# ScissorJack-ever/AlayaLite

Hardware: AMD Instinct MI355X
Metric: QPS @ recall@10>=0.95, GIST-960 L2, 1M base / 1k queries (higher is better)
Workload: dtype f32

## Files before the change

### alayalite_amd/csrc/capi.cpp

```cpp
#include "../../include/alaya_hip.h"

#include <hip/hip_runtime_api.h>

#include <algorithm>
#include <cfloat>
#include <cmath>
#include <cstring>
#include <memory>
#include <mutex>
#include <stdexcept>
#include <limits>
#include <string>
#include <thread>
#include <vector>

#include "build_kernels.h"
#include "extend_kernels.h"
#include "graph_update.h"
#include "hnsw_build.h"
#include "flat_bound.h"
#include "flat_filtered_kernels.h"
#include "flat_kernels.h"
#include <cstdlib>
#include "screen_bound.h"
// ... 33 lines not shown
    g_last_error = e.what();
    return ALAYA_ERR_DEVICE;
  } catch (const std::exception &e) {
    g_last_error = e.what();
    return ALAYA_ERR_RUNTIME;
  }
}

struct DevBuf {
  void *ptr = nullptr;
  size_t bytes = 0;
  void reserve(size_t n) {
    if (n <= bytes) return;
    release();
    hip_check(hipMalloc(&ptr, std::max<size_t>(n, 256)), "hipMalloc");
    bytes = std::max<size_t>(n, 256);
  }
  void release() {
    if (ptr) (void)hipFree(ptr);
    ptr = nullptr;
    bytes = 0;
  }
  template <typename T>
  T *as() const {
    return static_cast<T *>(ptr);
  }
  ~DevBuf() { release(); }
};

uint32_t round_up32(uint32_t d) { return (d + 31u) / 32u * 32u; }

uint32_t ceil_log2(uint64_t v) {
  uint32_t l = 0;
  while ((1ull << l) < v) ++l;
  return l;
}

}

struct alaya_index {
  int device = 0;
  std::mutex mu;
  uint64_t n = 0;
  uint32_t dim = 0, stride = 0;
  int metric = ALAYA_METRIC_L2;
  bool generic = false;
  DevBuf base, valid;
  bool has_valid = false;
  bool has_graph = false;
  uint32_t R = 0, upper_R = 0, ep = 0, n_eps = 0;
  bool has_overlay = false, dedup = false;
  DevBuf l0, levels, upper_off, upper_edges, eps;
  uint64_t graph_n = 0;
  bool has_sq8 = false;
  int sq8_order = 2;
  uint32_t code_stride = 0;
  DevBuf codes, sq_min, sq_max, rr_q_buf, sq_ids, sq_d;
  DevBuf norms, cand_d, cand_i, flat_tau, flag_buf, iota, flat_q;
  DevBuf flat_bias;
  int flat_contraction = -1;
  bool norms_ready = false;
  DevBuf flat_tiles, tiles_cand, tiles_qexp;
  bool tiles_ready = false;
  int tiles_exp = 0;
  int tiles_metric = -1;
  float max_norm = 0.f;
  DevBuf work, overflow, dirty, stab, q_buf, id_buf, dist_buf, cnt_buf, dlist_buf, dout_buf;
  DevBuf allow_buf, group_buf;
  DevBuf through_buf;
  DevBuf ff_ids, ff_sums, ff_count, ff_part_d, ff_part_i, ff_qlist;
  uint64_t ff_last[4] = {0, 0, 0, 0};
  size_t overflow_clean = 0;
  size_t stab_clean = 0;
  uint32_t hash_log2_override = 0;
  int helpers_mode = -1;
  DevBuf help_stats;
  uint64_t help_stats_slots = 0;
  struct ScreenCopy {
    DevBuf rows, err;
    uint64_t cap = 0;
    bool ready = false;
    bool failed = false;
  };
  ScreenCopy screen_copy[2];
  uint32_t screen_format = 0;
  DevBuf screen_stats;
  uint64_t screen_stats_slots = 0;
  uint32_t last_grid = 0, last_waves = 0;
  uint32_t last_lds = 0, last_hash_log2 = 0, last_compact = 0, last_per_cu = 0, last_scout = 0;
  DevBuf scout_stats;
  uint64_t scout_stats_slots = 0;
  DevBuf scout_policy_stats;
  uint32_t last_scout_policy = 0;
  int visited_mode_override = 0;
  int num_cus = 0;
  uint64_t capacity = 0;
  std::unique_ptr<alaya_amd::HostGraph> upd_graph;
  std::unique_ptr<alaya_amd::RowMirror> upd_rows;
  std::unique_ptr<alaya_amd::UpdateContext> upd_ctx;
  hipStream_t stream = nullptr;
  hipEvent_t scratch_ev = nullptr;
  hipStream_t scratch_stream = nullptr;
  bool scratch_used = false;
  uint64_t device_bytes() const {
    return base.bytes + valid.bytes + l0.bytes + levels.bytes + upper_off.bytes +
           upper_edges.bytes + eps.bytes + overflow.bytes + dirty.bytes + stab.bytes + codes.bytes + sq_min.bytes +
           sq_max.bytes;
  }
};

namespace {

void set_device(const alaya_index *ix) { hip_check(hipSetDevice(ix->device), "hipSetDevice"); }

void scratch_acquire(alaya_index *ix, hipStream_t s) {
  if (ix->scratch_used && ix->scratch_stream != s)
    hip_check(hipStreamWaitEvent(s, ix->scratch_ev, 0), "hipStreamWaitEvent");
}
void scratch_release(alaya_index *ix, hipStream_t s) {
  hip_check(hipEventRecord(ix->scratch_ev, s), "hipEventRecord");
  ix->scratch_stream = s;
  ix->scratch_used = true;
}
void scratch_suspect(alaya_index *ix) {
  ix->overflow_clean = 0;
  ix->stab_clean = 0;
}
void scratch_drain(alaya_index *ix) {
  if (!ix->scratch_used) return;
  const hipError_t e = hipEventSynchronize(ix->scratch_ev);
  if (e != hipSuccess) scratch_suspect(ix);
  hip_check(e, "hipEventSynchronize");
}
template <typename F>
int guarded_scratch(alaya_index *ix, F &&f) {
  return guarded([&] {
    try {
      f();
    } catch (const DeviceError &) {
      if (ix) scratch_suspect(ix);
      throw;
    }
  });
}

SearchParams base_params(alaya_index *ix) {
  SearchParams p{};
  p.base = ix->base.as<float>();
  p.n = ix->n;
  p.dim = ix->dim;
  p.stride = ix->stride;
  p.valid = ix->has_valid ? ix->valid.as<uint32_t>() : nullptr;
  p.ip = ix->metric != ALAYA_METRIC_L2;
  p.generic = ix->generic;
  return p;
}

constexpr size_t kLdsPerCu = 160 * 1024;
constexpr uint32_t kDirtyCap = 16384;

uint32_t spill_table_log2(int sq8_order, uint32_t L, uint32_t ef) {
  if (sq8_order != 2) return 0;
  uint32_t s = std::max<uint32_t>({6u, ceil_log2(32ull * ef), L > 12 ? L - 12 : 0u});
  if (const char *e = std::getenv("ALAYA_SPILL_TABLE")) {
    const uint32_t v = static_cast<uint32_t>(std::strtoul(e, nullptr, 10));
    if (v == 0) return 0;
    if (v >= 6 && v <= 16) s = v;
  }
  s = std::min<uint32_t>(s, L + 3);
  if (s > 16 || s < 6 || L - (s - 3) > 15) return 0;
// ... 178 lines not shown
  if (ensure_screen(ix, p, p.sq8_order == 0 && plain, stream)) r.want |= kModeScreen;
  return r;
}

struct SearchPlan {
  const alaya_amd::SearchVariant *variant;
  int W;
  size_t lds;
  int grid;
  int per_cu;
};

uint32_t scout_default(uint32_t dim) { return (dim == 768 || dim == 960) ? alaya_amd::kScoutOn : 0u; }

uint32_t scout_requested(uint32_t dim) {
  const char *e = std::getenv("ALAYA_SEARCH_SCOUT");
  const int asked = e && e[0] ? std::atoi(e) : -1;
  uint32_t f = asked < 0 ? scout_default(dim) : (asked == 1 ? alaya_amd::kScoutOn : (asked == 2 ? alaya_amd::kScoutOn | alaya_amd::kScoutVerify : 0u));
  if (f != 0u) {
    const char *m = std::getenv("ALAYA_SEARCH_SCOUT_MISS");
    if (m && std::atoi(m) != 0) f |= alaya_amd::kScoutMiss;
  }
  return f;
}

uint32_t scout_policy_default(uint32_t dim) {
  return (dim == 768 || dim == 960) ? (alaya_amd::kScoutEarly | alaya_amd::kScoutRecheck) : 0u;
}

uint32_t scout_policy_requested(uint32_t dim) {
  const char *e = std::getenv("ALAYA_SEARCH_SCOUT_POLICY");
  if (!(e && e[0])) return scout_policy_default(dim);
  return static_cast<uint32_t>(std::strtoul(e, nullptr, 0)) &
         (alaya_amd::kScoutEarly | alaya_amd::kScoutRecheck);
}

SearchPlan plan_search(alaya_index *ix, SearchParams &p, alaya_amd::SearchRequest r, uint64_t nq, uint32_t ef,
                       hipStream_t stream) {
  using namespace alaya_amd;
  SearchPlan plan{};
  for (;;) {
    plan.variant = &resolve_search_variant(r);
    const int mode = plan.variant->mode;
    if ((r.want & kModeStamp) != 0 && (mode & kModeStamp) == 0)
      throw ArgError("no stamped search kernel for dim " + std::to_string(ix->dim) +
                     (p.sq8_order ? " SQ8 (order " + std::to_string(p.sq8_order) + ")" : std::string(" f32")) +
                     ": see the variant list in search_variants.h");
    p.help = (mode & kModeHelp) != 0;
    p.two_waves = (mode & kModeTwoWaves) != 0;
    p.screen = (mode & kModeScreen) != 0 ? ix->screen_format : 0u;
    plan.W = p.help ? 4 : search_waves(p);
    while (!p.help && plan.W > 1 && static_cast<uint64_t>(plan.W) > nq) plan.W /= 2;
    p.hash_log2 = size_visited(ix, p, *plan.variant, nq, ef, plan.W);
    const bool compact = p.vis_rbits != kVisWide;
    p.wave_lds = static_cast<uint32_t>(search_wave_lds_bytes(ix->stride, ef, p.hash_log2, compact, p.sq8_order));
    bool fits = true;
    if (p.help) {
      const size_t need = static_cast<size_t>(plan.W) * kHelpMemoSlots * ix->R * 8;
      const size_t q_bytes = search_query_lds_bytes(ix->stride, p.sq8_order);
      if (q_bytes >= need) {
        p.memo_off = 0;
      } else if (p.wave_lds >= q_bytes + 3 * 64 * 4 + need) {
        p.memo_off = static_cast<uint32_t>(q_bytes + 3 * 64 * 4);
      } else {
        fits = false;
      }
    }
    plan.lds = search_shared_lds_bytes(ix->stride, p.sq8_order != 0) + static_cast<size_t>(plan.W) * p.wave_lds +
               (p.help ? kHelpBoardBytes : 0);
    if (!p.help || (fits && plan.lds <= kLdsPerCu)) break;
    r.want &= ~kModeHelp;
  }
  if (plan.lds > kLdsPerCu) throw ArgError("ef / dim too large for the LDS budget");
  int per_cu = 0;
  hip_check(search_occupancy(*plan.variant, p.ip, plan.W, plan.lds, &per_cu), "occupancy");
  per_cu = static_cast<int>(std::max<uint64_t>(1, std::min<uint64_t>(per_cu, max_search_waves_per_cu() / plan.W)));
  const uint64_t cus = static_cast<uint64_t>(stream_cus(ix, stream));
  const uint64_t blocks_needed = p.help ? static_cast<uint64_t>(per_cu) * cus : (nq + plan.W - 1) / plan.W;
  plan.grid = static_cast<int>(std::max<uint64_t>(1, std::min<uint64_t>(blocks_needed, static_cast<uint64_t>(per_cu) * cus)));
  plan.per_cu = per_cu;
  p.scout = 0u;
  p.scout_policy = 0u;
  const uint32_t scout = scout_requested(ix->dim);
  if (scout != 0u && p.screen == 3u && !p.ip && !p.two_waves && !p.help && plan.W == 1 && ix->R <= kScoutR &&
      (plan.variant->mode & ~kModeScreen) == 0 && search_has_two_waves(ix->dim, p.sq8_order, ix->generic) &&
      !helpers_requested(ix, p, nq, cus)) {
    SearchRequest r2 = r;
    r2.want |= kModeTwoWaves;
    const SearchVariant &v2 = resolve_search_variant(r2);
    const size_t lds2 = plan.lds + kScoutBoardBytes;
    int per_cu2 = 0;
    if (v2.mode == (kModeScreen | kModeTwoWaves) && lds2 <= kLdsPerCu)
      hip_check(search_occupancy(v2, false, 2, lds2, &per_cu2), "occupancy");
    if (per_cu2 >= per_cu && nq <= static_cast<uint64_t>(per_cu) * cus) {
      plan.variant = &v2;
      plan.lds = lds2;
      p.scout = scout;
      p.scout_policy = scout_policy_requested(ix->dim);
      if (const char *e = std::getenv("ALAYA_SEARCH_SCOUT_GRID"))
        plan.grid = std::max(1, std::min(plan.grid, std::atoi(e)));
    }
  }
  return plan;
}

SearchParams graph_search_params(alaya_index *ix, const float *d_q, uint64_t nq, uint32_t k, uint32_t ef, uint32_t *d_ids,
                                 float *d_dists, uint32_t *d_cnt) {
  SearchParams p = base_params(ix);
  p.l0 = ix->l0.as<uint32_t>();
  p.R = ix->R;
  p.dedup_edges = ix->dedup;
  p.levels = ix->has_overlay ? ix->levels.as<uint32_t>() : nullptr;
  p.upper_off = ix->upper_off.as<uint64_t>();
  p.upper_edges = ix->upper_edges.as<uint32_t>();
  p.upper_R = ix->upper_R;
  p.ep = ix->ep;
  p.eps = ix->eps.as<uint32_t>();
  p.n_eps = ix->n_eps;
  p.queries = d_q;
  p.nq = nq;
  p.q_stride = ix->dim;
  p.k = k;
  p.ef = ef;
  p.out_ids = d_ids;
  p.out_dists = d_dists;
  p.out_counters = d_cnt;
  return p;
}

void set_search_space(alaya_index *ix, SearchParams &p, bool sq8, uint32_t ef) {
  if (sq8) {
    p.sq8_order = ix->sq8_order;
    p.codes = ix->codes.as<uint8_t>();
    p.code_stride = ix->code_stride;
    p.sq_min = ix->sq_min.as<float>();
    p.sq_max = ix->sq_max.as<float>();
  }
  p.stab_log2 = spill_table_log2(p.sq8_order, std::max<uint32_t>(1, ceil_log2(std::max<uint64_t>(ix->n, 2))), ef);
}

void record_launch(alaya_index *ix, SearchParams &p, int grid, int wg_waves, size_t lds, int per_cu, uint64_t searchers,
                   hipStream_t stream) {
  ix->last_grid = static_cast<uint32_t>(grid);
  ix->last_waves = static_cast<uint32_t>(wg_waves);
  ix->last_lds = static_cast<uint32_t>(lds);
  ix->last_hash_log2 = p.hash_log2;
  ix->last_compact = p.vis_rbits != alaya_amd::kVisWide ? 1u : 0u;
  ix->last_per_cu = static_cast<uint32_t>(per_cu);
  ix->last_scout = p.scout;
  ix->last_scout_policy = p.scout_policy;
  ix->scout_stats_slots = p.scout ? searchers : 0;
  ix->help_stats_slots = p.help ? searchers : 0;
  ix->screen_stats_slots = p.screen ? searchers : 0;
  ix->work.reserve(4);
  p.work_counter = ix->work.as<uint32_t>();
  hip_check(hipMemsetAsync(p.work_counter, 0, 4, stream), "hipMemsetAsync");
}

void do_search(alaya_index *ix, const float *d_q, uint64_t nq, uint32_t k, uint32_t ef,
               uint32_t *d_ids, float *d_dists, uint32_t *d_cnt, hipStream_t stream,
               uint64_t *d_stamps = nullptr, bool sq8 = false, uint32_t fill_id = 0) {
  if (!ix->base.ptr) throw ArgError("index has no base vectors");
  if (!ix->has_graph) throw ArgError("index has no graph");
  if (ef == 0) throw ArgError("ef must be >= 1");
  if (k == 0 || nq == 0) return;
  if (ix->graph_n > ix->n) throw ArgError("graph has more nodes than base vectors");
  SearchParams p = graph_search_params(ix, d_q, nq, k, ef, d_ids, d_dists, d_cnt);
  p.stamps = d_stamps;
  p.fill_id = fill_id;
  if (sq8 && !ix->has_sq8) throw ArgError("index has no SQ8 codes");
  set_search_space(ix, p, sq8, ef);
  if (const char *e = std::getenv("ALAYA_HELP_FLAGS")) p.help_flags = static_cast<uint32_t>(std::strtoul(e, nullptr, 10));
  const SearchPlan plan = plan_search(ix, p, search_request(ix, p, nq, ef, stream), nq, ef, stream);
  if (p.screen >= 2) {
    p.screen_u8 = ix->screen_copy[1].rows.as<uint8_t>();
  } else if (p.screen) {
    p.screen_rows = ix->screen_copy[0].rows.as<uint16_t>();
    p.screen_err = ix->screen_copy[0].err.as<float>();
  }
  scratch_acquire(ix, stream);
  const uint64_t searchers = static_cast<uint64_t>(plan.grid) * plan.W;
  prepare_spill(ix, p, searchers, stream);
  const int wg_waves = p.scout ? 2 * plan.W : plan.W;
  if (p.scout) {
    ix->scout_stats.reserve(searchers * 16);
    p.scout_stats = ix->scout_stats.as<uint32_t>();
    ix->scout_policy_stats.reserve(searchers * 12);
    p.scout_policy_stats = ix->scout_policy_stats.as<uint32_t>();
  }
  if (p.help) {
    ix->help_stats.reserve(searchers * 12);
    p.help_stats = ix->help_stats.as<uint32_t>();
  }
  if (p.screen) {
    ix->screen_stats.reserve(searchers * 8);
    p.screen_stats = ix->screen_stats.as<uint32_t>();
  }
  record_launch(ix, p, plan.grid, wg_waves, plan.lds, plan.per_cu, searchers, stream);
  hip_check(alaya_amd::launch_search(*plan.variant, p, plan.grid, wg_waves, plan.lds, stream), "search launch");
  scratch_release(ix, stream);
}

void do_filtered_search(alaya_index *ix, const float *d_q, uint64_t nq, uint32_t k, uint32_t ef, const uint32_t *d_allow,
                        const uint32_t *d_mask_of_query, uint32_t *d_ids, float *d_dists, uint32_t *d_cnt,
                        hipStream_t stream, bool sq8 = false, bool hop = false, uint32_t *d_through = nullptr) {
  using namespace alaya_amd;
  if (hop && (sq8 || ix->has_sq8))
    throw ArgError("through search of an SQ8 index: alaya_index_filtered_search_hop searches f32 rows only");
  if (!ix->base.ptr) throw ArgError("index has no base vectors");
  if (!ix->has_graph) throw ArgError("index has no graph");
  if (sq8 && !ix->has_sq8) throw ArgError("index has no SQ8 codes");
  if (!sq8 && ix->has_sq8)
    throw ArgError("filtered search of an SQ8 index: use alaya_index_filtered_search_sq8 (this call searches f32 rows only)");
  if (ef == 0) throw ArgError("ef must be >= 1");
  if (k == 0 || k > 224) throw ArgError("filtered search: k must be in 1..224");
  if (nq == 0) return;
  if (ix->graph_n > ix->n) throw ArgError("graph has more nodes than base vectors");
  SearchParams p = graph_search_params(ix, d_q, nq, k, ef, d_ids, d_dists, d_cnt);
  p.fill_id = 0xffffffffu;
  set_search_space(ix, p, sq8, ef);
  const SearchVariant &plain = resolve_search_variant({ix->dim, p.ip, p.sq8_order, ix->generic, 0});
  int W = search_waves(p);
  while (W > 1 && static_cast<uint64_t>(W) > nq) W /= 2;
  p.hash_log2 = size_visited(ix, p, plain, nq, ef, W, k, hop);
  const size_t traversal_lds = search_wave_lds_bytes(ix->stride, ef, p.hash_log2, p.vis_rbits != kVisWide, p.sq8_order);
  p.wave_lds = static_cast<uint32_t>(traversal_lds + filter_result_lds_bytes(k));
  FilterParams f{};
  f.allow = d_allow;
  f.mask_of_query = d_mask_of_query;
  f.mask_words = static_cast<uint32_t>((ix->n + 31) / 32);
  f.k = k;
  f.result_off = static_cast<uint32_t>(traversal_lds);
  const size_t lds = search_shared_lds_bytes(ix->stride, sq8) + static_cast<size_t>(W) * p.wave_lds;
  if (lds > kLdsPerCu) throw ArgError("filtered search: k / ef / dim too large for the LDS budget");
  int per_cu = 0;
  hip_check(sq8 ? filtered_sq8_search_occupancy(ix->dim, p.sq8_order, p.ip, W, lds, &per_cu)
            : hop ? filtered_hop_search_occupancy(ix->dim, ix->generic, p.ip, W, lds, &per_cu)
                : filtered_search_occupancy(ix->dim, ix->generic, p.ip, W, lds, &per_cu),
            "occupancy");
  per_cu = static_cast<int>(std::max<uint64_t>(1, std::min<uint64_t>(per_cu, max_search_waves_per_cu() / W)));
  const uint64_t cus = static_cast<uint64_t>(stream_cus(ix, stream));
  int grid = static_cast<int>(std::max<uint64_t>(1, std::min<uint64_t>((nq + W - 1) / W, static_cast<uint64_t>(per_cu) * cus)));
  if (const char *e = std::getenv("ALAYA_FILTER_GRID")) grid = std::max(1, std::min(grid, std::atoi(e)));
  scratch_acquire(ix, stream);
  const uint64_t searchers = static_cast<uint64_t>(grid) * W;
  prepare_spill(ix, p, searchers, stream);
  record_launch(ix, p, grid, W, lds, per_cu, searchers, stream);
  hip_check(sq8   ? launch_filtered_sq8_search(p, f, grid, W, lds, stream)
            : hop ? launch_filtered_hop_search(p, f, HopParams{d_through}, grid, W, lds, stream)
                  : launch_filtered_search(p, f, grid, W, lds, stream),
            "filtered search launch");
  scratch_release(ix, stream);
}

uint32_t screen_default(uint32_t dim) {
  return (dim == 512 || dim == 768 || dim == 960 || dim == 1024) ? 3u : 0u;
}

void screen_fill(alaya_index *ix, uint32_t format, uint64_t first, uint64_t count, hipStream_t stream) {
  alaya_index::ScreenCopy &c = ix->screen_copy[format - 1];
  hip_check(format == 2 ? alaya_amd::launch_screen_rows_u8(ix->base.as<float>(), first, count, ix->stride,
                                                           c.rows.as<uint8_t>(), stream)
                        : alaya_amd::launch_screen_rows(ix->base.as<float>(), first, count, ix->stride,
                                                        c.rows.as<uint16_t>(), c.err.as<float>(), stream),
            "screening copy");
}

bool ensure_screen(alaya_index *ix, const SearchParams &p, bool eligible, hipStream_t stream) {
  ix->screen_format = 0;
  if (!eligible || !alaya_amd::search_has_screen(ix->dim, p.sq8_order, ix->generic, p.ip)) return false;
  const char *e = std::getenv("ALAYA_SEARCH_SCREEN");
  const int asked = e && e[0] ? std::atoi(e) : -1;
  const uint32_t format =
      asked < 0 ? screen_default(ix->dim) : (asked == 0 ? 0u : (asked == 9 ? 3u : (asked == 8 ? 2u : 1u)));
  if (format == 0) return false;
  const uint32_t copy = format == 3 ? 2u : format;
  alaya_index::ScreenCopy &c = ix->screen_copy[copy - 1];
  if (c.failed) return false;
  if (!c.ready) {
    const uint64_t rows = std::max<uint64_t>(std::max(ix->capacity, ix->n), 1);
    try {
      if (rows > c.cap) {
        c.rows.release();
        c.err.release();
        c.cap = 0;
        if (copy == 2) {
          c.rows.reserve(rows * alaya_amd::screen_u8_record_bytes(ix->stride));
        } else {
          c.rows.reserve(rows * ix->stride * 2);
          c.err.reserve(rows * 4);
        }
        c.cap = rows;
      }
    } catch (const DeviceError &) {
      (void)hipGetLastError();
      c.rows.release();
      c.err.release();
      c.cap = 0;
      c.failed = true;
      return false;
    }
    scratch_acquire(ix, stream);
    screen_fill(ix, copy, 0, ix->n, stream);
    c.ready = true;
  }
  ix->screen_format = format;
  return true;
}

void screen_drop(alaya_index *ix) {
  for (alaya_index::ScreenCopy &c : ix->screen_copy) {
    c.rows.release();
    c.err.release();
    c.cap = 0;
    c.ready = false;
    c.failed = false;
  }
  ix->screen_format = 0;
  ix->screen_stats_slots = 0;
}

void ensure_norms(alaya_index *ix, hipStream_t stream) {
  if (ix->norms_ready) return;
  ix->norms.reserve(std::max<uint64_t>(ix->n, 1) * 4);
  hip_check(alaya_amd::launch_row_norms(ix->base.as<float>(), ix->n, ix->stride, ix->norms.as<float>(), stream),
            "row norms");
  std::vector<float> h(ix->n);
  hip_check(hipMemcpyAsync(h.data(), ix->norms.ptr, ix->n * 4, hipMemcpyDeviceToHost, stream), "D2H");
  hip_check(hipStreamSynchronize(stream), "norms");
  float mx = 0.f;
  for (float v : h) mx = std::max(mx, v);
  ix->max_norm = std::sqrt(mx) * 1.0001f;
  if (ix->metric != ALAYA_METRIC_L2) {
    ix->flat_bias.reserve(std::max<uint64_t>(ix->n, 1) * 4);
    hip_check(hipMemsetAsync(ix->flat_bias.ptr, 0, std::max<uint64_t>(ix->n, 1) * 4, stream), "flat bias");
  }
  ix->norms_ready = true;
}

int flat_chunks(alaya_index *ix, int nqg, uint64_t rows) {
  int chunks = (ix->num_cus + nqg - 1) / nqg;
  chunks = std::max(8, (chunks + 7) / 8 * 8);
  const uint64_t max_chunks = std::max<uint64_t>(8, (rows / 64) / 8 * 8);
  return static_cast<int>(std::min<uint64_t>(chunks, max_chunks));
}

int flat_tiles_chunks(alaya_index *ix, uint64_t nq, uint64_t scan_tiles) {
  const uint64_t qpb = alaya_amd::flat_tiles_queries();
  const uint64_t nqg = (nq + qpb - 1) / qpb;
  const uint64_t cus = static_cast<uint64_t>(std::max(1, ix->num_cus));
  const uint64_t cap = std::max<uint64_t>(8, std::min<uint64_t>(256, (scan_tiles / 4) / 8 * 8));
  if (nqg * 8 < cus) return static_cast<int>(std::min<uint64_t>(cap, (cus + nqg - 1) / nqg + 7) / 8 * 8);
  uint64_t best = 8;
  double best_eff = 0.0;
  for (uint64_t c = 8; c <= std::min<uint64_t>(64, cap); c += 8) {
    const uint64_t b = nqg * c;
    const double eff = static_cast<double>(b) / static_cast<double>((b + cus - 1) / cus * cus);
    if (eff > best_eff + 1e-9) {
      best_eff = eff;
      best = c;
    }
  }
  return static_cast<int>(best);
}

const float *flat_bias(const alaya_index *ix) {
  return ix->metric == ALAYA_METRIC_L2 ? ix->norms.as<float>() : ix->flat_bias.as<float>();
}

void ensure_tiles(alaya_index *ix, int base_exp, hipStream_t stream) {
  if (ix->tiles_ready && ix->tiles_exp == base_exp && ix->tiles_metric == ix->metric) return;
  const size_t bytes = alaya_amd::flat_tiles_bytes(ix->stride, ix->n);
  ix->flat_tiles.reserve(std::max<size_t>(bytes, 256));
  hip_check(alaya_amd::launch_flat_tiles(ix->base.as<float>(), ix->n, ix->stride, flat_bias(ix),
                                         ix->has_valid ? ix->valid.as<uint32_t>() : nullptr, base_exp,
                                         ix->flat_tiles.as<unsigned char>(), stream),
            "flat tile records");
  ix->tiles_ready = true;
  ix->tiles_exp = base_exp;
  ix->tiles_metric = ix->metric;
}

void flat_prescan(alaya_index *ix, alaya_amd::FlatParams &p, hipStream_t s) {
  const char *env = std::getenv("ALAYA_FLAT_PRESCAN");
  const uint64_t step = env ? std::strtoull(env, nullptr, 10) : 0;
  auto sample_scan = [&](alaya_amd::FlatParams q, int nqg) {
    q.tau_init = nullptr;
    q.out_ids = nullptr;
    q.out_dists = nullptr;
    q.flags = nullptr;
    q.merge_count = nullptr;
    q.ablate = 0;
    ix->flat_tau.reserve(p.nq * 4);
    q.tau_out = ix->flat_tau.as<float>();
    hip_check(alaya_amd::launch_flat_scan(q, nqg * q.n_chunks, s), "flat prescan");
    hip_check(alaya_amd::launch_flat_threshold(q, s), "flat threshold");
    p.tau_init = q.tau_out;
  };
  if (p.tiles != nullptr) {
    const uint64_t nt = p.n_scan_tiles;
    const char *genv = std::getenv("ALAYA_FLAT_PRESCAN_GROUPS");
    const char *senv = std::getenv("ALAYA_FLAT_PRESCAN_SAMPLE");
// ... 434 lines not shown
        hip_check(hipMemcpyAsync(b.ptr, src, bytes, hipMemcpyHostToDevice, ix->stream), "upload graph");
    };
    bool dup = false;
    for (uint64_t i = 0; i < h.n && !dup; ++i) {
      const uint32_t *r = &h.l0[i * h.R];
      for (uint32_t a = 0; a < h.R && r[a] != 0xffffffffu && !dup; ++a)
        for (uint32_t b = 0; b < a; ++b)
          if (r[a] == r[b]) {
            dup = true;
            break;
          }
    }
    up(ix->l0, h.l0.data(), h.l0.size() * 4);
    up(ix->levels, h.levels.data(), h.levels.size() * 4);
    up(ix->upper_off, h.upper_off.data(), h.upper_off.size() * 8);
    up(ix->upper_edges, h.upper_edges.data(), h.upper_edges.size() * 4);
    up(ix->eps, h.eps.data(), h.eps.size() * 4);
    hip_check(hipStreamSynchronize(ix->stream), "sync");
    ix->R = h.R;
    ix->upper_R = h.upper_R;
    ix->ep = h.ep;
    ix->n_eps = static_cast<uint32_t>(h.eps.size());
    ix->has_overlay = h.has_overlay;
    ix->dedup = dup;
    ix->graph_n = h.n;
    ix->has_graph = true;
    ix->upd_graph.reset();
    ix->upd_rows.reset();
    ix->upd_ctx.reset();
  });
}

namespace {

void grow_keep(alaya_index *ix, DevBuf &b, size_t bytes, size_t keep) {
  if (bytes <= b.bytes) return;
  DevBuf nb;
  nb.reserve(bytes);
  hip_check(hipMemsetAsync(nb.ptr, 0, nb.bytes, ix->stream), "memset");
  if (keep && b.ptr) hip_check(hipMemcpyAsync(nb.ptr, b.ptr, keep, hipMemcpyDeviceToDevice, ix->stream), "copy");
  hip_check(hipStreamSynchronize(ix->stream), "sync");
  std::swap(b.ptr, nb.ptr);
  std::swap(b.bytes, nb.bytes);
}

void reserve_locked(alaya_index *ix, uint64_t capacity) {
  if (!ix->base.ptr) throw ArgError("index has no base vectors");
  if (capacity < ix->n) throw ArgError("capacity below the stored rows");
  const size_t row = static_cast<size_t>(ix->stride) * 4;
  grow_keep(ix, ix->base, std::max<uint64_t>(capacity, 1) * row, ix->n * row);
  const size_t words = (std::max<uint64_t>(capacity, 1) + 31) / 32;
  if (!ix->has_valid) {
    std::vector<uint32_t> w(words, 0u);
    for (uint64_t i = 0; i < ix->n; ++i) w[i >> 5] |= 1u << (i & 31);
    ix->valid.release();
    ix->valid.reserve(words * 4);
    hip_check(hipMemcpyAsync(ix->valid.ptr, w.data(), words * 4, hipMemcpyHostToDevice, ix->stream), "bitmap");
    hip_check(hipStreamSynchronize(ix->stream), "sync");
    ix->has_valid = true;
  } else {
    grow_keep(ix, ix->valid, words * 4, (ix->n + 31) / 32 * 4);
  }
  if (ix->has_graph) {
    grow_keep(ix, ix->l0, std::max<uint64_t>(capacity, 1) * ix->R * 4, ix->graph_n * ix->R * 4);
    grow_keep(ix, ix->levels, std::max<uint64_t>(capacity, 1) * 4, ix->graph_n * 4);
    grow_keep(ix, ix->upper_off, std::max<uint64_t>(capacity, 1) * 8, ix->graph_n * 8);
  }
  ix->capacity = std::max(ix->capacity, capacity);
}

void write_rows_locked(alaya_index *ix, uint64_t first, const float *rows, uint64_t count) {
  scratch_drain(ix);
  const size_t row = static_cast<size_t>(ix->stride) * 4;
  if (first + count > ix->capacity || (first + count) * row > ix->base.bytes)
    throw ArgError("rows beyond the reserved capacity");
  char *dst = static_cast<char *>(ix->base.ptr) + first * row;
  hip_check(hipMemset2DAsync(dst, row, 0, row, count, ix->stream), "memset");
  hip_check(hipMemcpy2DAsync(dst, row, rows, static_cast<size_t>(ix->dim) * 4, static_cast<size_t>(ix->dim) * 4,
                             count, hipMemcpyHostToDevice, ix->stream), "write rows");
  hip_check(hipStreamSynchronize(ix->stream), "sync");
  ix->n = std::max(ix->n, first + count);
  ix->norms_ready = false;
  ix->tiles_ready = false;
  for (uint32_t format = 1; format <= 2; ++format) {
    alaya_index::ScreenCopy &c = ix->screen_copy[format - 1];
    if (!c.ready) continue;
    if (first + count <= c.cap) {
      screen_fill(ix, format, first, count, ix->stream);
      hip_check(hipStreamSynchronize(ix->stream), "sync");
    } else {
      c.ready = false;
    }
  }
}

void write_edges_locked(alaya_index *ix, const uint32_t *ids, const uint32_t *edges, uint64_t count) {
  if (!ix->has_graph) throw ArgError("index has no graph");
  scratch_drain(ix);
  for (uint64_t i = 0; i < count; ++i) {
    if (ids[i] >= ix->capacity || ids[i] >= ix->n || (static_cast<uint64_t>(ids[i]) + 1) * ix->R * 4 > ix->l0.bytes ||
        (ix->has_overlay && (static_cast<uint64_t>(ids[i]) + 1) * 4 > ix->levels.bytes))
      throw ArgError("edge row id out of range (reserve capacity first)");
    const uint32_t *r = edges + i * ix->R;
    for (uint32_t a = 0; a < ix->R && r[a] != 0xffffffffu; ++a) {
      for (uint32_t b = 0; b < a; ++b)
        if (r[a] == r[b]) ix->dedup = true;
    }
    hip_check(hipMemcpyAsync(ix->l0.as<uint32_t>() + static_cast<uint64_t>(ids[i]) * ix->R, r, ix->R * 4,
                             hipMemcpyHostToDevice, ix->stream), "write edges");
    ix->graph_n = std::max<uint64_t>(ix->graph_n, static_cast<uint64_t>(ids[i]) + 1);
  }
  hip_check(hipStreamSynchronize(ix->stream), "sync");
}

void set_valid_locked(alaya_index *ix, uint64_t id, bool valid) {
  if (!ix->has_valid || id >= ix->capacity || (id / 32 + 1) * 4 > ix->valid.bytes)
    throw ArgError("id out of range (reserve capacity first)");
  scratch_drain(ix);
  uint32_t w = 0;
  uint32_t *dw = ix->valid.as<uint32_t>() + (id >> 5);
  hip_check(hipMemcpy(&w, dw, 4, hipMemcpyDeviceToHost), "read bitmap");
  w = valid ? (w | (1u << (id & 31))) : (w & ~(1u << (id & 31)));
  hip_check(hipMemcpy(dw, &w, 4, hipMemcpyHostToDevice), "write bitmap");
  ix->tiles_ready = false;
}

}

int alaya_index_reserve(alaya_index *ix, uint64_t capacity) {
  return guarded([&] {
    if (!ix) throw ArgError("invalid arguments");
    std::lock_guard<std::mutex> lk(ix->mu);
    set_device(ix);
    scratch_drain(ix);
    reserve_locked(ix, capacity);
  });
}

int alaya_index_write_rows(alaya_index *ix, uint64_t first, const float *rows, uint64_t count) {
  return guarded([&] {
    if (!ix || (count && !rows)) throw ArgError("invalid arguments");
    std::lock_guard<std::mutex> lk(ix->mu);
    set_device(ix);
    write_rows_locked(ix, first, rows, count);
  });
}

int alaya_index_write_edges(alaya_index *ix, const uint32_t *ids, const uint32_t *edges, uint64_t count) {
  return guarded([&] {
    if (!ix || (count && (!ids || !edges))) throw ArgError("invalid arguments");
    std::lock_guard<std::mutex> lk(ix->mu);
    set_device(ix);
    write_edges_locked(ix, ids, edges, count);
  });
}

int alaya_index_set_valid(alaya_index *ix, uint64_t id, int valid) {
  return guarded([&] {
    if (!ix) throw ArgError("invalid arguments");
    std::lock_guard<std::mutex> lk(ix->mu);
    set_device(ix);
    set_valid_locked(ix, id, valid != 0);
  });
}

int alaya_index_enable_updates(alaya_index *ix, const alaya_graph *g, const float *rows, uint64_t n,
                               uint64_t capacity, const uint8_t *valid_bitmap) {
// ... 1247 lines not shown
  return guarded_scratch(ix, [&] {
    if (!ix) throw ArgError("null index");
    const std::vector<uint64_t> t = searcher_stats(ix, ix->help_stats, ix->help_stats_slots, 3);
    if (memo_dists) *memo_dists = t[0];
    if (memo_expansions) *memo_expansions = t[1];
    if (helper_rows) *helper_rows = t[2];
  });
}

int alaya_screen_lower_bound(const float *d_tilde, const float *e_row, uint64_t n, uint32_t dim, float *out) {
  return guarded([&] {
    if (n && (!d_tilde || !e_row || !out)) throw ArgError("invalid arguments");
    for (uint64_t i = 0; i < n; ++i) out[i] = alaya_amd::screen_lower_bound(d_tilde[i], e_row[i], dim);
  });
}

namespace {
void screen_u8_quantize_one(const float *x, uint32_t dim, uint8_t *codes, float *header, float *values) {
  using namespace alaya_amd;
  float lo = FLT_MAX, hi = -FLT_MAX;
  bool bad = false;
  for (uint32_t j = 0; j < dim; ++j) {
    bad = bad || !screen_finite(x[j]);
    lo = fminf(lo, x[j]);
    hi = fmaxf(hi, x[j]);
  }
  float scale = screen_u8_scale(lo, hi);
  if (bad || !screen_finite(scale)) {
    bad = true;
    lo = scale = 0.f;
  }
  float sum = 0.f;
  for (uint32_t j = 0; j < dim; ++j) {
    const uint32_t c = screen_u8_code(x[j], lo, scale);
    const float y = screen_u8_value(c, lo, scale);
    const float d = x[j] - y;
    if (!bad) sum = fmaf(d, d, sum);
    codes[j] = static_cast<uint8_t>(c);
    if (values) values[j] = y;
  }
  header[0] = screen_u8_err(sum, dim, bad);
  header[1] = lo;
  header[2] = scale;
  header[3] = 0.f;
}
}

int alaya_screen_u8_quantize(const float *rows, uint64_t n, uint32_t dim, uint8_t *codes, float *header,
                             float *values) {
  return guarded([&] {
    if (n && dim && (!rows || !codes || !header || !values)) throw ArgError("invalid arguments");
    for (uint64_t r = 0; r < n; ++r)
      screen_u8_quantize_one(rows + r * dim, dim, codes + r * dim, header + 4 * r, values + r * dim);
  });
}

int alaya_screen_int_bound(const float *queries, const float *rows, uint64_t n, uint32_t dim, float *d_in,
                           float *e_sum, float *bound, uint32_t *sums) {
  return guarded([&] {
    using namespace alaya_amd;
    if (dim == 0 || dim > 4096) throw ArgError("dim must be in 1 .. 4096");
    if (n && (!queries || !rows || !d_in || !e_sum || !bound || !sums)) throw ArgError("invalid arguments");
    std::vector<uint8_t> a(dim), c(dim);
    for (uint64_t i = 0; i < n; ++i) {
      float qh[4], rh[4];
      screen_u8_quantize_one(queries + i * dim, dim, a.data(), qh, nullptr);
      screen_u8_quantize_one(rows + i * dim, dim, c.data(), rh, nullptr);
      uint32_t a1 = 0, a2 = 0, c1 = 0, c2 = 0, ac = 0;
      for (uint32_t j = 0; j < dim; ++j) {
        const uint32_t aj = a[j], cj = c[j];
        a1 += aj; a2 += aj * aj;
        c1 += cj; c2 += cj * cj;
        ac += aj * cj;
      }
      d_in[i] = screen_int_distance(dim, qh[1], qh[2], a1, a2, rh[1], rh[2], c1, c2, ac);
      e_sum[i] = screen_int_err(rh[0], rh[1], rh[2], qh[0], qh[1], qh[2]);
      bound[i] = screen_int_bound(dim, qh[0], qh[1], qh[2], a1, a2, rh[0], rh[1], rh[2], c1, c2, ac);
      uint32_t *s = sums + 5 * i;
      s[0] = a1; s[1] = a2; s[2] = c1; s[3] = c2; s[4] = ac;
    }
  });
}

int alaya_flat_ip_slack(int contraction, uint32_t k_acc, const float *q_norm2, const int *q_exp, uint64_t n,
                        float b_max, int base_exp, float *out) {
  return guarded([&] {
    if (contraction < 0 || contraction > 2 || (n && (!q_norm2 || !out))) throw ArgError("invalid arguments");
    for (uint64_t i = 0; i < n; ++i)
      out[i] = alaya_amd::flat_ip_slack(contraction, k_acc, q_norm2[i], q_exp ? q_exp[i] : 0, b_max, base_exp);
  });
}

int alaya_flat_ip_proven(const float *kth_d, const float *cutoff, const float *slack, uint64_t n, uint8_t *out) {
  return guarded([&] {
    if (n && (!kth_d || !cutoff || !slack || !out)) throw ArgError("invalid arguments");
    for (uint64_t i = 0; i < n; ++i) out[i] = alaya_amd::flat_ip_proven(kth_d[i], cutoff[i], slack[i]) ? 1 : 0;
  });
}

int alaya_search_variant(uint32_t dim, int ip, int sq8_order, int generic, uint32_t wanted_mode, int *space,
                         uint32_t *chunks, uint32_t *mode, uint32_t *has_mode) {
  return guarded([&] {
    using namespace alaya_amd;
    if (sq8_order < 0 || sq8_order > 2 || wanted_mode >= 32u) throw ArgError("invalid arguments");
    const SearchVariant &v = resolve_search_variant({dim, ip != 0, sq8_order, generic != 0, static_cast<int>(wanted_mode)});
    if (space) *space = v.space;
    if (chunks) *chunks = static_cast<uint32_t>(v.chunks);
    if (mode) *mode = static_cast<uint32_t>(v.mode);
    if (has_mode)
      *has_mode = (search_has_helpers(dim, sq8_order, generic != 0) ? kModeHelp : 0) |
                  (search_has_two_waves(dim, sq8_order, generic != 0) ? kModeTwoWaves : 0) |
                  (search_has_screen(dim, sq8_order, generic != 0, ip != 0) ? kModeScreen : 0);
  });
}

int alaya_search_variant_at(uint32_t index, int *space, uint32_t *chunks, uint32_t *mode, int *l2_only,
                            uint32_t *count) {
  return guarded([&] {
    if (count) *count = static_cast<uint32_t>(alaya_amd::kNumSearchVariants);
    if (index >= alaya_amd::kNumSearchVariants) throw ArgError("variant index out of range");
    const alaya_amd::SearchVariant &v = alaya_amd::kSearchVariants[index];
    if (space) *space = v.space;
    if (chunks) *chunks = static_cast<uint32_t>(v.chunks);
    if (mode) *mode = static_cast<uint32_t>(v.mode);
    if (l2_only) *l2_only = v.l2_only ? 1 : 0;
  });
}

int alaya_index_screen_stats(alaya_index *ix, uint64_t *screened, uint64_t *screened_out) {
  return guarded_scratch(ix, [&] {
    if (!ix) throw ArgError("null index");
    const std::vector<uint64_t> t = searcher_stats(ix, ix->screen_stats, ix->screen_stats_slots, 2);
    if (screened) *screened = t[0];
    if (screened_out) *screened_out = t[1];
  });
}

int alaya_index_set_visited_mode(alaya_index *ix, int mode) {
  return guarded([&] {
    if (!ix) throw ArgError("null index");
    if (mode < 0 || mode > 3) throw ArgError("visited mode must be 0 (auto), 1 (compact), 2 (wide) or 3 (test)");
    ix->visited_mode_override = mode;
  });
}

int alaya_index_info(const alaya_index *ix, uint64_t *n, uint32_t *dim, uint32_t *stride,
                     int *metric, uint64_t *device_bytes) {
  return guarded([&] {
    if (!ix) throw ArgError("null index");
    if (n) *n = ix->n;
    if (dim) *dim = ix->dim;
    if (stride) *stride = ix->stride;
    if (metric) *metric = ix->metric;
    if (device_bytes) *device_bytes = ix->device_bytes();
  });
}

}
```

### alayalite_amd/csrc/pybind_module.cpp

```cpp
#include <pybind11/numpy.h>
#include <pybind11/pybind11.h>
#include <pybind11/stl.h>

#include <algorithm>
#include <cmath>
#include <cstring>
#include <fstream>
#include <memory>
#include <queue>
#include <stdexcept>
#include <string>
#include <vector>

#include "../../include/alaya_hip.h"

extern "C" int alaya_index_flat_diag(alaya_index *, const float *, uint64_t, uint32_t, int, uint32_t *, float *,
                                     uint32_t *, uint32_t *, void *);
#include "host_distance.h"

namespace py = pybind11;

namespace alaya_py {

enum class IndexType { FLAT = 0, HNSW = 1, NSG = 2, FUSION = 3, QG = 4 };
// ... 46 lines not shown
  if (allow_words.ndim() != 2 || static_cast<uint64_t>(allow_words.shape(1)) != (n + 31) / 32 || allow_words.shape(0) < 1)
    throw py::value_error("allow_words must be uint32 [n_masks, ceil(n / 32)]");
  Masks m;
  m.words = allow_words.data();
  m.n_masks = static_cast<uint32_t>(allow_words.shape(0));
  if (!mask_of_query.is_none()) {
    m.indices = U32Array(mask_of_query);
    if (m.indices.ndim() != 1 || static_cast<uint64_t>(m.indices.shape(0)) != nq)
      throw py::value_error("mask_of_query must hold one index per query");
    m.of_query = m.indices.data();
  }
  return m;
}

enum DType { kF32 = 0, kI8, kU8, kF64, kI32, kU32 };

DType dtype_code(const py::dtype &dt) {
  if (dt.is(py::dtype::of<float>())) return kF32;
  if (dt.is(py::dtype::of<int8_t>())) return kI8;
  if (dt.is(py::dtype::of<uint8_t>())) return kU8;
  if (dt.is(py::dtype::of<double>())) return kF64;
  if (dt.is(py::dtype::of<int32_t>())) return kI32;
  if (dt.is(py::dtype::of<uint32_t>())) return kU32;
  throw std::runtime_error("Unsupported data type");
}

size_t dtype_size(DType t) {
  switch (t) {
    case kF32: case kI32: case kU32: return 4;
    case kI8: case kU8: return 1;
    case kF64: return 8;
  }
  return 4;
}

void to_float(const void *src, DType t, size_t count, float *dst) {
  switch (t) {
    case kF32: std::memcpy(dst, src, count * 4); break;
    case kI8: for (size_t i = 0; i < count; ++i) dst[i] = static_cast<const int8_t *>(src)[i]; break;
    case kU8: for (size_t i = 0; i < count; ++i) dst[i] = static_cast<const uint8_t *>(src)[i]; break;
    case kF64: for (size_t i = 0; i < count; ++i) dst[i] = static_cast<float>(static_cast<const double *>(src)[i]); break;
    case kI32: for (size_t i = 0; i < count; ++i) dst[i] = static_cast<float>(static_cast<const int32_t *>(src)[i]); break;
    case kU32: for (size_t i = 0; i < count; ++i) dst[i] = static_cast<float>(static_cast<const uint32_t *>(src)[i]); break;
  }
}

int host_sq8_order() { return __builtin_cpu_supports("avx512f") ? 2 : 1; }

py::tuple graph_arrays_of(const alaya_graph *g) {
  uint64_t n, nue;
  uint32_t R, upper_R, ep, max_level, n_eps;
  int has_overlay;
  check(alaya_graph_info(g, &n, &R, &has_overlay, &upper_R, &ep, &max_level, &nue, &n_eps));
  py::array_t<uint32_t> l0 = out2d<uint32_t>(n, R);
  py::array_t<uint32_t> levels(static_cast<py::ssize_t>(has_overlay ? n : 0));
  py::array_t<uint64_t> off(static_cast<py::ssize_t>(has_overlay ? n : 0));
  py::array_t<uint32_t> ue(static_cast<py::ssize_t>(nue));
  py::array_t<uint32_t> eps(static_cast<py::ssize_t>(n_eps));
  check(alaya_graph_export(g, l0.mutable_data(), levels.mutable_data(), off.mutable_data(), ue.mutable_data(),
                           eps.mutable_data()));
  return py::make_tuple(l0, has_overlay ? py::object(levels) : py::none(), has_overlay ? py::object(off) : py::none(), ue,
                        ep, upper_R, eps);
}

class LaunchControls {
 public:
  void set_hash_log2(uint32_t v) { check(alaya_index_set_hash_log2(ix_, v)); }
  void set_visited_mode(int m) { check(alaya_index_set_visited_mode(ix_, m)); }
  void set_helpers(int m) { check(alaya_index_set_helpers(ix_, m)); }
  py::tuple last_launch() {
    uint32_t g = 0, w = 0;
    check(alaya_index_last_launch(ix_, &g, &w));
    return py::make_tuple(g, w);
  }
  py::tuple help_stats() {
    uint64_t m = 0, x = 0, r = 0;
    check(alaya_index_help_stats(ix_, &m, &x, &r));
    return py::make_tuple(m, x, r);
  }
  py::tuple screen_stats() {
    uint64_t a = 0, b = 0;
    check(alaya_index_screen_stats(ix_, &a, &b));
    return py::make_tuple(a, b);
  }
  py::tuple scout_stats() {
    uint64_t e = 0, h = 0, r = 0, m = 0;
    check(alaya_index_scout_stats(ix_, &e, &h, &r, &m));
    return py::make_tuple(e, h, r, m);
  }
  py::tuple scout_policy_stats() {
    uint64_t a = 0, c = 0, d = 0;
    check(alaya_index_scout_policy_stats(ix_, nullptr, &a, &c, &d));
    return py::make_tuple(a, c, d);
  }
  uint32_t scout_policy() {
    uint32_t pol = 0;
    check(alaya_index_scout_policy_stats(ix_, &pol, nullptr, nullptr, nullptr));
    return pol;
  }
  py::dict last_plan() {
    uint32_t g = 0, w = 0, lds = 0, hl = 0, c = 0, pc = 0, sc = 0;
    check(alaya_index_last_launch(ix_, &g, &w));
    check(alaya_index_last_plan(ix_, &lds, &hl, &c, &pc, &sc));
    py::dict d;
    d["workgroups"] = g;
    d["waves_per_group"] = w;
    d["lds_bytes"] = lds;
    d["hash_log2"] = hl;
    d["compact"] = c != 0;
    d["groups_per_cu"] = pc;
    d["scout"] = sc;
    d["scout_policy"] = scout_policy();
    return d;
  }

 protected:
  alaya_index *ix_ = nullptr;
};

class PyIndexInterface : public LaunchControls {
 public:
  explicit PyIndexInterface(const IndexParams &params) : params_(params) {
    dtype_ = dtype_code(params_.data_type_);
    if (params_.id_type_.is(py::dtype::of<uint32_t>())) {
      id_bytes_ = 4;
    } else if (params_.id_type_.is(py::dtype::of<uint64_t>())) {
      id_bytes_ = 8;
    } else {
      throw std::runtime_error("Unsupported id type");
    }
    if (params_.quantization_type_ == QuantizationType::SQ4 ||
        params_.quantization_type_ == QuantizationType::RABITQ)
      throw std::runtime_error("quantization type not supported by the MI355X engine (SQ4/RaBitQ are out of scope)");
    if (params_.metric_ == MetricType::COS && dtype_ != kF32 && dtype_ != kF64) {
      throw std::runtime_error("COS metric only support float or double");
    }
    if (params_.quantization_type_ == QuantizationType::SQ8 && dtype_ != kF32)
      throw std::runtime_error("SQ8 quantization of non-float32 data is not supported by the MI355X engine");
    check(alaya_index_create(0, &ix_));
  }
  ~PyIndexInterface() {
    if (graph_) alaya_graph_free(graph_);
    if (ix_) alaya_index_destroy(ix_);
  }
  PyIndexInterface(const PyIndexInterface &) = delete;
  PyIndexInterface &operator=(const PyIndexInterface &) = delete;

  std::string to_string() const { return "PyIndexInterface"; }

  void fit(py::array vectors, uint32_t ef_construction, uint32_t num_threads, const std::string &builder) {
    if (builder != "host" && builder != "gpu") throw py::value_error("builder must be 'host' or 'gpu'");
    if (vectors.ndim() != 2) throw std::runtime_error("Array must be 2D");
    check_dtype(vectors);
    py::array arr = py::array::ensure(vectors, py::array::c_style);
    const uint64_t n = arr.shape(0);
    dim_ = static_cast<uint32_t>(arr.shape(1));
    if (n > params_.capacity_) throw std::runtime_error("number of vectors exceeds the index capacity");
    if (params_.metric_ == MetricType::COS) normalize_in_place(arr, n);
    raw_.assign(static_cast<const char *>(arr.data()),
                static_cast<const char *>(arr.data()) + n * dim_ * dtype_size(dtype_));
    n_ = n;
    delete_cnt_ = 0;
    valid_.clear();
    rows_f32_.resize(n * dim_);
    to_float(raw_.data(), dtype_, n * dim_, rows_f32_.data());
    if (graph_) alaya_graph_free(graph_);
// ... 885 lines not shown
  using namespace alaya_py;
  m.doc() = "AlayaLite MI355X engine";
  m.attr("__version__") = "0.1.0-mi355x";

  py::enum_<IndexType>(m, "IndexType")
      .value("FLAT", IndexType::FLAT)
      .value("HNSW", IndexType::HNSW)
      .value("NSG", IndexType::NSG)
      .value("FUSION", IndexType::FUSION)
      .export_values();
  py::enum_<MetricType>(m, "MetricType")
      .value("L2", MetricType::L2)
      .value("IP", MetricType::IP)
      .value("COS", MetricType::COS)
      .export_values();
  py::enum_<QuantizationType>(m, "QuantizationType")
      .value("NONE", QuantizationType::NONE)
      .value("SQ8", QuantizationType::SQ8)
      .value("SQ4", QuantizationType::SQ4)
      .value("RABITQ", QuantizationType::RABITQ)
      .export_values();

  py::class_<IndexParams>(m, "IndexParams")
      .def(py::init<>())
      .def(py::init([](IndexType it, py::dtype dt, py::dtype idt, QuantizationType qt, MetricType mt,
                       uint32_t cap) {
             IndexParams p;
             p.index_type_ = it;
             p.data_type_ = std::move(dt);
             p.id_type_ = std::move(idt);
             p.quantization_type_ = qt;
             p.metric_ = mt;
             p.capacity_ = cap;
             return p;
           }),
           py::arg("index_type_") = IndexType::HNSW, py::arg("data_type_") = py::dtype::of<float>(),
           py::arg("id_type_") = py::dtype::of<uint32_t>(),
           py::arg("quantization_type_") = QuantizationType::NONE,
           py::arg("metric_") = MetricType::L2, py::arg("capacity_") = 100000u)
      .def_readwrite("index_type_", &IndexParams::index_type_)
      .def_readwrite("data_type_", &IndexParams::data_type_)
      .def_readwrite("id_type_", &IndexParams::id_type_)
      .def_readwrite("quantization_type_", &IndexParams::quantization_type_)
      .def_readwrite("metric_", &IndexParams::metric_)
      .def_readwrite("capacity_", &IndexParams::capacity_);

  py::class_<PyIndexInterface, std::shared_ptr<PyIndexInterface>>(m, "PyIndexInterface")
      .def(py::init<IndexParams>(), py::arg("params"))
      .def("to_string", &PyIndexInterface::to_string)
      .def("fit", &PyIndexInterface::fit, py::arg("vectors"), py::arg("ef_construction"), py::arg("num_threads"),
           py::arg("builder") = "host")
      .def("search", &PyIndexInterface::search, py::arg("query"), py::arg("topk"), py::arg("ef"))
      .def("get_data_by_id", &PyIndexInterface::get_data_by_id, py::arg("id"))
      .def("insert", &PyIndexInterface::insert, py::arg("insert_data"), py::arg("ef"))
      .def("remove", &PyIndexInterface::remove, py::arg("id"))
      .def("add", &PyIndexInterface::add, py::arg("vectors"), py::arg("ef_construction"))
      .def("sq8_codes", &PyIndexInterface::sq8_codes)
      .def("sq8_range", &PyIndexInterface::sq8_range)
      .def("last_build_device_ms", &PyIndexInterface::last_build_device_ms)
      .def("batch_search", &PyIndexInterface::batch_search, py::arg("queries"), py::arg("topk"),
           py::arg("ef"), py::arg("num_threads"))
      .def("batch_search_with_distance", &PyIndexInterface::batch_search_with_distance,
           py::arg("queries"), py::arg("topk"), py::arg("ef"), py::arg("num_threads"))
      .def("exact_search", &PyIndexInterface::exact_search, py::arg("queries"), py::arg("topk"))
      .def("exact_search_filtered", &PyIndexInterface::exact_search_filtered, py::arg("queries"), py::arg("topk"),
           py::arg("allow_words"), py::arg("mask_of_query") = py::none())
      .def("save", &PyIndexInterface::save, py::arg("index_path"), py::arg("data_path"),
           py::arg("quant_path") = std::string())
      .def("load", &PyIndexInterface::load, py::arg("index_path"), py::arg("data_path"),
           py::arg("quant_path") = std::string())
      .def("filtered_search", &PyIndexInterface::filtered_search, py::arg("queries"), py::arg("topk"), py::arg("ef"),
           py::arg("allow_words"), py::arg("mask_of_query") = py::none(), py::arg("pool") = 0,
           py::arg("through") = false)
      .def("last_through", &PyIndexInterface::last_through)
      .def("get_data_dim", &PyIndexInterface::get_data_dim)
      .def("get_data_num", &PyIndexInterface::get_data_num)
      .def("last_counters", &PyIndexInterface::last_counters)
      .def("set_hash_log2", &PyIndexInterface::set_hash_log2)
      .def("set_visited_mode", &PyIndexInterface::set_visited_mode)
      .def("set_helpers", &PyIndexInterface::set_helpers)
      .def("last_launch", &PyIndexInterface::last_launch)
      .def("help_stats", &PyIndexInterface::help_stats)
      .def("screen_stats", &PyIndexInterface::screen_stats)
      .def("scout_stats", &PyIndexInterface::scout_stats)
      .def("scout_policy_stats", &PyIndexInterface::scout_policy_stats)
      .def("last_plan", &PyIndexInterface::last_plan)
      .def("set_rerank_mode", &PyIndexInterface::set_rerank_mode)
      .def("rerank_mode", &PyIndexInterface::rerank_mode)
      .def("device_distances", &PyIndexInterface::device_distances)
      .def("graph_arrays", &PyIndexInterface::graph_arrays);


  py::class_<Graph, std::shared_ptr<Graph>>(m, "Graph")
      .def_static("build", &Graph::build, py::arg("data"), py::arg("metric") = 0, py::arg("R") = 32u,
                  py::arg("ef_construction") = 100u, py::arg("num_threads") = 1u, py::arg("seed") = 100u)
      .def_static("load", &Graph::load, py::arg("path"), py::arg("id_bytes") = 4)
      .def_static("from_arrays", &Graph::from_arrays, py::arg("l0"), py::arg("levels"), py::arg("upper_off"),
                  py::arg("upper_edges"), py::arg("upper_R"), py::arg("ep"), py::arg("eps") = py::none())
      .def("save", &Graph::save, py::arg("path"), py::arg("id_bytes") = 4, py::arg("capacity") = 0u)
      .def("arrays", &Graph::arrays);
  py::class_<DeviceIndex, std::shared_ptr<DeviceIndex>>(m, "DeviceIndex")
      .def(py::init<int>(), py::arg("device") = 0)
      .def("set_base", &DeviceIndex::set_base, py::arg("rows"), py::arg("metric") = 0, py::arg("valid") = py::none())
      .def("set_graph", &DeviceIndex::set_graph)
      .def("build_graph", &DeviceIndex::build_graph, py::arg("R") = 32, py::arg("ef_construction") = 100,
           py::arg("seed") = 100, py::arg("batch_div") = 0, py::arg("max_batch") = 0, py::arg("refine") = 2)
      .def("extend_graph", &DeviceIndex::extend_graph, py::arg("rows"), py::arg("ef_construction") = 100,
           py::arg("seed") = 100, py::arg("batch_div") = 0, py::arg("max_batch") = 0, py::arg("refine") = 2)
      .def("read_sq8", &DeviceIndex::read_sq8, py::arg("first"), py::arg("count"))
      .def("search", &DeviceIndex::search, py::arg("queries"), py::arg("k"), py::arg("ef"))
      .def("search_device", &DeviceIndex::search_device)
      .def("filtered_search", &DeviceIndex::filtered_search, py::arg("queries"), py::arg("k"), py::arg("ef"),
           py::arg("allow_words"), py::arg("mask_of_query") = py::none())
      .def("filtered_search_device", &DeviceIndex::filtered_search_device)
      .def("filtered_search_hop", &DeviceIndex::filtered_search_hop, py::arg("queries"), py::arg("k"), py::arg("ef"),
           py::arg("allow_words"), py::arg("mask_of_query") = py::none())
      .def("filtered_search_hop_device", &DeviceIndex::filtered_search_hop_device)
      .def("filtered_search_sq8", &DeviceIndex::filtered_search_sq8, py::arg("queries"), py::arg("k"), py::arg("ef"),
           py::arg("allow_words"), py::arg("mask_of_query") = py::none(), py::arg("pool") = 0,
           py::arg("rerank_queries") = py::none())
      .def("filtered_search_sq8_device", &DeviceIndex::filtered_search_sq8_device)
      .def("shard_search_device", &DeviceIndex::shard_search_device)
      .def("distances", &DeviceIndex::distances)
      .def("set_hash_log2", &DeviceIndex::set_hash_log2)
      .def("set_visited_mode", &DeviceIndex::set_visited_mode)
      .def("set_helpers", &DeviceIndex::set_helpers)
      .def("last_launch", &DeviceIndex::last_launch)
      .def("help_stats", &DeviceIndex::help_stats)
      .def("screen_stats", &DeviceIndex::screen_stats)
      .def("scout_stats", &DeviceIndex::scout_stats)
      .def("scout_policy_stats", &DeviceIndex::scout_policy_stats)
      .def("last_plan", &DeviceIndex::last_plan)
      .def("flat_search", &DeviceIndex::flat_search, py::arg("queries"), py::arg("k"))
      .def("flat_search_device", &DeviceIndex::flat_search_device)
      .def("flat_search_filtered", &DeviceIndex::flat_search_filtered, py::arg("queries"), py::arg("k"),
           py::arg("allow_words"), py::arg("mask_of_query") = py::none())
      .def("flat_search_filtered_device", &DeviceIndex::flat_search_filtered_device)
      .def("flat_filtered_last", &DeviceIndex::flat_filtered_last)
      .def("flat_diag", &DeviceIndex::flat_diag)
      .def("flat_contraction", &DeviceIndex::flat_contraction)
      .def("search_sq8_device", &DeviceIndex::search_sq8_device)
      .def("shard_search_sq8_device", &DeviceIndex::shard_search_sq8_device)
      .def("set_sq8", &DeviceIndex::set_sq8, py::arg("codes"), py::arg("min"), py::arg("max"), py::arg("order") = 2)
      .def("search_sq8", &DeviceIndex::search_sq8, py::arg("queries"), py::arg("k"), py::arg("ef"),
           py::arg("rerank") = 1, py::arg("rerank_queries") = py::none())
      .def("profile_search", &DeviceIndex::profile_search, py::arg("q"), py::arg("k"), py::arg("ef"),
           py::arg("space") = 0)
      .def("device_bytes", &DeviceIndex::device_bytes);
  m.def("sq8_train", [](F32Array data) {
    const uint32_t d = static_cast<uint32_t>(data.shape(1));
    py::array_t<float> mn(d), mx(d);
    check(alaya_sq8_train(data.data(), data.shape(0), d, mn.mutable_data(), mx.mutable_data()));
    return py::make_tuple(mn, mx);
  });
  m.def("sq8_encode", [](F32Array data, F32Array mn, F32Array mx, uint32_t threads) {
    py::array_t<uint8_t> codes({data.shape(0), data.shape(1)});
    check(alaya_sq8_encode(data.data(), data.shape(0), static_cast<uint32_t>(data.shape(1)), mn.data(), mx.data(),
                           codes.mutable_data(), threads));
    return codes;
  }, py::arg("data"), py::arg("min"), py::arg("max"), py::arg("num_threads") = 1u);
  m.def("host_sq8_order", &host_sq8_order);
  m.def("build_batches", [](U32Array levels, uint64_t start, uint32_t ep, uint32_t batch_div, uint32_t max_batch) {
    if (levels.ndim() != 1) throw py::value_error("levels must be 1D");
    const uint64_t n = levels.shape(0);
    uint64_t nb = 0;
    check(alaya_build_batches(levels.data(), n, start, ep, batch_div, max_batch, nullptr, &nb));
    py::array_t<uint64_t> ends(static_cast<py::ssize_t>(nb));
    check(alaya_build_batches(levels.data(), n, start, ep, batch_div, max_batch, ends.mutable_data(), &nb));
    return ends;
  }, py::arg("levels"), py::arg("start") = 1, py::arg("ep") = 0, py::arg("batch_div") = 0, py::arg("max_batch") = 0);
  m.def("build_info", [] { return std::string(alaya_build_info()); });
  m.def("screen_lower_bound", [](F32Array d_tilde, F32Array e_row, uint32_t dim) {
    if (d_tilde.size() != e_row.size()) throw std::invalid_argument("d_tilde and e_row differ in size");
    py::array_t<float> out(d_tilde.size());
    check(alaya_screen_lower_bound(d_tilde.data(), e_row.data(), static_cast<uint64_t>(d_tilde.size()), dim,
                                   out.mutable_data()));
    return out;
  });
  m.def("screen_u8_quantize", [](F32Array rows) {
    if (rows.ndim() != 2) throw std::invalid_argument("rows must be 2-D");
    py::array_t<uint8_t> codes({rows.shape(0), rows.shape(1)});
    py::array_t<float> header({rows.shape(0), static_cast<py::ssize_t>(4)});
    py::array_t<float> values({rows.shape(0), rows.shape(1)});
    check(alaya_screen_u8_quantize(rows.data(), static_cast<uint64_t>(rows.shape(0)), static_cast<uint32_t>(rows.shape(1)),
                                   codes.mutable_data(), header.mutable_data(), values.mutable_data()));
    return py::make_tuple(codes, header, values);
  });
  m.def("screen_int_bound", [](F32Array queries, F32Array rows) {
    if (rows.ndim() != 2 || queries.ndim() != 2 || rows.shape(0) != queries.shape(0) || rows.shape(1) != queries.shape(1))
      throw std::invalid_argument("queries and rows must be 2-D of one shape");
    py::array_t<float> d_in(rows.shape(0)), e_sum(rows.shape(0)), bound(rows.shape(0));
    py::array_t<uint32_t> sums({rows.shape(0), static_cast<py::ssize_t>(5)});
    check(alaya_screen_int_bound(queries.data(), rows.data(), static_cast<uint64_t>(rows.shape(0)),
                                 static_cast<uint32_t>(rows.shape(1)), d_in.mutable_data(), e_sum.mutable_data(),
                                 bound.mutable_data(), sums.mutable_data()));
    return py::make_tuple(d_in, e_sum, bound, sums);
  });
  m.def("flat_filtered_plan", [](uint64_t n_allowed, uint64_t nq, uint32_t k, uint32_t stride, uint32_t cus) {
    uint64_t o[5] = {0, 0, 0, 0, 0};
    check(alaya_flat_filtered_plan(n_allowed, nq, k, stride, cus, o));
    return py::make_tuple(o[0], o[1], o[2], o[3], o[4]);
  }, py::arg("n_allowed"), py::arg("nq"), py::arg("k"), py::arg("stride"), py::arg("cus"));
  m.def("flat_ip_slack", [](int contraction, uint32_t k_acc, F32Array q_norm2, CArray<int> q_exp, float b_max,
                            int base_exp) {
    if (q_exp.size() != 0 && q_exp.size() != q_norm2.size()) throw std::invalid_argument("q_norm2 and q_exp differ in size");
    py::array_t<float> out(q_norm2.size());
    check(alaya_flat_ip_slack(contraction, k_acc, q_norm2.data(), q_exp.size() ? q_exp.data() : nullptr,
                              static_cast<uint64_t>(q_norm2.size()), b_max, base_exp, out.mutable_data()));
    return out;
  }, py::arg("contraction"), py::arg("k_acc"), py::arg("q_norm2"), py::arg("q_exp"), py::arg("b_max"),
     py::arg("base_exp") = 0);
  m.def("flat_ip_proven", [](F32Array kth_d, F32Array cutoff, F32Array slack) {
    if (kth_d.size() != cutoff.size() || kth_d.size() != slack.size()) throw std::invalid_argument("sizes differ");
    py::array_t<uint8_t> out(kth_d.size());
    check(alaya_flat_ip_proven(kth_d.data(), cutoff.data(), slack.data(), static_cast<uint64_t>(kth_d.size()),
                               out.mutable_data()));
    return out;
  }, py::arg("kth_d"), py::arg("cutoff"), py::arg("slack"));
  m.def("normalize_rows", [](F32Array a) {
    if (a.ndim() != 2) throw std::invalid_argument("normalize_rows needs a 2D array");
    py::array_t<float> out({a.shape(0), a.shape(1)});
    if (a.size()) std::memcpy(out.mutable_data(), a.data(), static_cast<size_t>(a.size()) * 4);
    for (py::ssize_t i = 0; i < a.shape(0); ++i)
      alaya_amd::normalize_row(out.mutable_data() + i * a.shape(1), static_cast<size_t>(a.shape(1)));
    return out;
  }, py::arg("array"));
  m.def("search_variant", [](uint32_t dim, bool ip, int sq8_order, bool generic, uint32_t wanted_mode) {
    int space = 0;
    uint32_t chunks = 0, mode = 0, has = 0;
    check(alaya_search_variant(dim, ip, sq8_order, generic, wanted_mode, &space, &chunks, &mode, &has));
    return py::make_tuple(py::make_tuple(space, chunks, mode), has);
  }, py::arg("dim"), py::arg("ip"), py::arg("sq8_order"), py::arg("generic"), py::arg("wanted_mode"));
  m.def("search_variants", [] {
    py::list rows;
    uint32_t count = 1;
    for (uint32_t i = 0; i < count; ++i) {
      int space = 0, l2_only = 0;
      uint32_t chunks = 0, mode = 0;
      check(alaya_search_variant_at(i, &space, &chunks, &mode, &l2_only, &count));
      rows.append(py::make_tuple(space, chunks, mode, l2_only != 0));
    }
    return rows;
  });
  m.def("device_count", [] {
    int c = 0;
    check(alaya_device_count(&c));
    return c;
  });
  m.def("hbm_stream_read", [](int device, uint64_t bytes, int iters) {
    double gbs = 0.0;
    check(alaya_hbm_stream_read(device, bytes, iters, &gbs));
    return gbs;
  }, py::arg("device") = 0, py::arg("bytes") = 4ull << 30, py::arg("iters") = 5);
  m.def("stream_create_reserving", [](int device, uint32_t reserved_cus) {
    void *s = nullptr;
    check(alaya_stream_create_reserving(device, reserved_cus, &s));
    return reinterpret_cast<uintptr_t>(s);
  }, py::arg("device"), py::arg("reserved_cus"));
  m.def("stream_destroy", [](uintptr_t s) { check(alaya_stream_destroy(dptr<void>(s))); });
}
```

### alayalite_amd/csrc/screen_bound.h

```cpp
#pragma once
#include <cmath>
#include <cstdint>

#if defined(__HIPCC__) || defined(__CUDACC__)
#define ALAYA_HD __host__ __device__
#else
#define ALAYA_HD
#endif

namespace alaya_amd {

ALAYA_HD inline float screen_gamma(uint32_t dim) { return static_cast<float>(dim + 16u) * 5.9604644775390625e-8f; }

constexpr float kScreenTiny = 8.271806125530277e-25f;
constexpr float kScreenHuge = 1.2676506002282294e30f;

ALAYA_HD inline float screen_lower_bound(float d_tilde, float e_row, uint32_t dim) {
  if (!(d_tilde >= kScreenTiny) || !(d_tilde <= kScreenHuge)) return 0.f;
  if (!(e_row >= 0.f) || !(e_row <= kScreenHuge)) return 0.f;
  const float keep = 1.0f - screen_gamma(dim);
  const float y = d_tilde * keep;
  const float s = sqrtf(y) * (1.0f - 9.5367431640625e-7f);
  const float t = s - e_row;
  if (!(t > 0.f)) return 0.f;
  const float r = (t * t) * keep;
  return r >= kScreenTiny ? r : 0.f;
}

constexpr uint32_t kScreenU8Header = 16;
ALAYA_HD inline uint32_t screen_u8_record_bytes(uint32_t stride) { return (kScreenU8Header + stride + 63u) & ~63u; }

ALAYA_HD inline float screen_u8_value(uint32_t c, float lo, float scale) {
  return fmaf(static_cast<float>(c), scale, lo);
}

ALAYA_HD inline float screen_u8_scale(float lo, float hi) { return (hi - lo) / 255.0f; }
ALAYA_HD inline uint32_t screen_u8_code(float x, float lo, float scale) {
  if (!(scale > 0.f)) return 0u;
  const float c = rintf((x - lo) / scale);
  return c >= 255.f ? 255u : (c >= 0.f ? static_cast<uint32_t>(c) : 0u);
}

ALAYA_HD inline float screen_u8_err(float sum, uint32_t stride, bool bad) {
  const float err = sqrtf(sum * (1.0f + screen_gamma(stride))) * (1.0f + 1.9073486328125e-6f) + 8.8817841970012523e-16f;
  return (bad || !(err <= kScreenHuge)) ? INFINITY : err;
}
ALAYA_HD inline bool screen_finite(float x) { return fabsf(x) <= 3.4028234663852886e38f; }

ALAYA_HD inline uint32_t screen_u8_sums_offset(uint32_t stride) { return kScreenU8Header + stride; }

ALAYA_HD inline float screen_int_distance(uint32_t n, float qlo, float qs, uint32_t a1, uint32_t a2, float lo,
                                          float s, uint32_t c1, uint32_t c2, uint32_t ac) {
  const double delta = static_cast<double>(qlo) - static_cast<double>(lo);
  const double dq = qs, dr = s;
  const double t1 = (static_cast<double>(n) * delta) * delta;
  const double t2 = (2.0 * delta) * (dq * static_cast<double>(a1));
  const double t3 = (2.0 * delta) * (dr * static_cast<double>(c1));
  const double t4 = (dq * dq) * static_cast<double>(a2);
  const double t5 = (dr * dr) * static_cast<double>(c2);
  const double t6 = (2.0 * (dq * dr)) * static_cast<double>(ac);
  const double sum = ((t1 + t4) + t5) + ((t2 - t3) - t6);
  const double mag = ((t1 + t4) + t5) + ((fabs(t2) + fabs(t3)) + t6);
  const double d = (sum - mag * 1.7763568394002505e-15) * (1.0 - 1.1920928955078125e-7);
  if (!(d > 0.0) || !(d <= static_cast<double>(kScreenHuge))) return 0.f;
  return static_cast<float>(d);
}

ALAYA_HD inline float screen_int_err(float e_row, float lo, float s, float e_q, float qlo, float qs) {
  const double m_row = fmax(fabs(static_cast<double>(lo)), fabs(static_cast<double>(lo) + 255.0 * static_cast<double>(s)));
  const double m_q = fmax(fabs(static_cast<double>(qlo)), fabs(static_cast<double>(qlo) + 255.0 * static_cast<double>(qs)));
  const double e = ((static_cast<double>(e_row) + static_cast<double>(e_q)) + ((m_row + m_q) * 3.814697265625e-6 +
                                                                            7.888609052210118e-31)) *
                   (1.0 + 2.384185791015625e-7);
  return static_cast<float>(e);
}

ALAYA_HD inline float screen_int_bound(uint32_t n, float e_q, float qlo, float qs, uint32_t a1, uint32_t a2, float e_row,
                                       float lo, float s, uint32_t c1, uint32_t c2, uint32_t ac) {
  return screen_lower_bound(screen_int_distance(n, qlo, qs, a1, a2, lo, s, c1, c2, ac),
                            screen_int_err(e_row, lo, s, e_q, qlo, qs), n);
}

}
```

### alayalite_amd/csrc/search_device.h

```cpp
#pragma once
#include <hip/hip_runtime.h>

#include <cfloat>
#include <cstdint>

#include "screen_bound.h"
#include "search_kernels.h"

namespace alaya_amd {
namespace {

constexpr uint32_t kEmpty = 0xffffffffu;
constexpr uint32_t kChecked = 0x80000000u;
constexpr uint32_t kIdMask = 0x7fffffffu;

__device__ __forceinline__ int lane_id() { return __lane_id(); }

__device__ __forceinline__ void wave_sync() {
  __builtin_amdgcn_fence(__ATOMIC_SEQ_CST, "wavefront");
  __builtin_amdgcn_wave_barrier();
}

__device__ __forceinline__ uint64_t ballot(bool p) { return __ballot(p); }

// ... 492 lines not shown
  Q.err = screen_u8_err(read_lane(sum, 0) + read_lane(sum, 32), p.stride, bad);
  return Q;
}

template <int kXor, int kN>
__device__ __forceinline__ void screen_fold(uint32_t *v, bool upper) {
#pragma unroll
  for (int i = 0; i < kN / 2; ++i) {
    const uint32_t keep = upper ? v[i + kN / 2] : v[i];
    const uint32_t send = upper ? v[i] : v[i + kN / 2];
    v[i] = keep + lane_xor<kXor>(send);
  }
}

__device__ __forceinline__ int screen_pass_row(int lane) {
  return ((lane & 1) << 4) | ((lane & 2) << 2) | (lane & 4) | ((lane & 8) >> 2) | ((lane & 16) >> 4);
}

template <int kChunks, typename Hook>
__device__ __forceinline__ uint32_t screen_dots_pass(const SearchParams &p, const uint4 qc, uint32_t id, Hook after_issue) {
  constexpr int kPieces = 2 * kChunks;
  const int lane = lane_id();
  const uint32_t rec = screen_u8_record_bytes(p.stride);
  const uint32_t piece = kScreenU8Header + 16u * static_cast<uint32_t>(lane < kPieces ? lane : kPieces - 1);
  uint4 y[32];
#pragma unroll
  for (int r = 0; r < 32; ++r) {
    const uint8_t *rp = p.screen_u8 + static_cast<uint64_t>(read_lane(id, r)) * rec;
    y[r] = *reinterpret_cast<const uint4 *>(rp + piece);
  }
  __builtin_amdgcn_sched_barrier(0);
  after_issue();
  uint32_t acc[32];
#pragma unroll
  for (int r = 0; r < 32; ++r) {
    uint32_t a = __builtin_amdgcn_udot4(qc.x, y[r].x, 0u, false);
    a = __builtin_amdgcn_udot4(qc.y, y[r].y, a, false);
    a = __builtin_amdgcn_udot4(qc.z, y[r].z, a, false);
    acc[r] = __builtin_amdgcn_udot4(qc.w, y[r].w, a, false);
    if ((r & 7) == 7) __builtin_amdgcn_sched_barrier(0);
  }
  screen_fold<1, 32>(acc, (lane & 1) != 0);
  screen_fold<2, 16>(acc, (lane & 2) != 0);
  screen_fold<4, 8>(acc, (lane & 4) != 0);
  screen_fold<8, 4>(acc, (lane & 8) != 0);
  screen_fold<16, 2>(acc, (lane & 16) != 0);
  return acc[0] + static_cast<uint32_t>(__builtin_amdgcn_ds_bpermute((lane ^ 32) << 2, static_cast<int>(acc[0])));
}

template <int kChunks, typename Hook>
__device__ __forceinline__ void screen_dots_int(const SearchParams &p, const uint4 qc, const uint32_t *ids, int n,
                                                uint32_t *out, Hook after_issue) {
  constexpr int kPieces = 2 * kChunks;
  const int lane = lane_id();
  const uint32_t rec = screen_u8_record_bytes(p.stride);
  const uint32_t piece = kScreenU8Header + 16u * static_cast<uint32_t>(lane < kPieces ? lane : kPieces - 1);
  const int mine = ((lane & 1) << 4) | ((lane & 2) << 2) | (lane & 4) | ((lane & 8) >> 2) | ((lane & 16) >> 4);
  for (int base = 0; base < n; base += 32) {
    const uint32_t id = ids[base + lane < n ? base + lane : base];
    uint4 y[32];
#pragma unroll
    for (int r = 0; r < 32; ++r) {
      const uint8_t *rp = p.screen_u8 + static_cast<uint64_t>(read_lane(id, r)) * rec;
      y[r] = *reinterpret_cast<const uint4 *>(rp + piece);
    }
    __builtin_amdgcn_sched_barrier(0);
    if (base == 0) after_issue();
    uint32_t acc[32];
#pragma unroll
    for (int r = 0; r < 32; ++r) {
      uint32_t a = __builtin_amdgcn_udot4(qc.x, y[r].x, 0u, false);
      a = __builtin_amdgcn_udot4(qc.y, y[r].y, a, false);
      a = __builtin_amdgcn_udot4(qc.z, y[r].z, a, false);
      acc[r] = __builtin_amdgcn_udot4(qc.w, y[r].w, a, false);
      if ((r & 7) == 7) __builtin_amdgcn_sched_barrier(0);
    }
    screen_fold<1, 32>(acc, (lane & 1) != 0);
    screen_fold<2, 16>(acc, (lane & 2) != 0);
    screen_fold<4, 8>(acc, (lane & 4) != 0);
    screen_fold<8, 4>(acc, (lane & 8) != 0);
    screen_fold<16, 2>(acc, (lane & 16) != 0);
    const uint32_t tot = acc[0] + static_cast<uint32_t>(__builtin_amdgcn_ds_bpermute((lane ^ 32) << 2, static_cast<int>(acc[0])));
    if (lane < 32 && base + mine < n) out[base + mine] = tot;
  }
  wave_sync();
}

template <bool kIP>
__device__ __forceinline__ float sq8_term(float xq, float scale, float mn, float yf, float acc) {
  if (kIP) return fmaf(xq, fmaf(yf, scale, mn), acc);
  const float d = (xq - yf) * scale;
  return fmaf(d, d, acc);
}

#ifndef ALAYA_SQ8_QCODES
#define ALAYA_SQ8_QCODES 0
#endif
template <int kOrder>
constexpr bool sq8_query_codes() { return ALAYA_SQ8_QCODES != 0 && kOrder == 2; }

template <bool kIP, bool kCodes>
__device__ __forceinline__ float4 sq8_qterm4(const float *xq, const float4 &s, const float4 &mn, int e) {
  if constexpr (!kCodes) {
    return *reinterpret_cast<const float4 *>(xq + e);
  } else {
    const uint32_t w = *reinterpret_cast<const uint32_t *>(reinterpret_cast<const uint8_t *>(xq) + e);
    const float c0 = static_cast<float>(w & 0xffu), c1 = static_cast<float>((w >> 8) & 0xffu);
    const float c2 = static_cast<float>((w >> 16) & 0xffu), c3 = static_cast<float>(w >> 24);
    if (kIP) return make_float4(fmaf(c0, s.x, mn.x), fmaf(c1, s.y, mn.y), fmaf(c2, s.z, mn.z), fmaf(c3, s.w, mn.w));
    return make_float4(c0, c1, c2, c3);
  }
}
template <bool kIP, bool kCodes>
__device__ __forceinline__ float sq8_qterm(const float *xq, const float *sc, const float *mnv, int e) {
  if constexpr (!kCodes) return xq[e];
  const float c = static_cast<float>(reinterpret_cast<const uint8_t *>(xq)[e]);
  return kIP ? fmaf(c, sc[e], mnv[e]) : c;
}

template <bool kIP, bool kCodes = false>
__device__ __forceinline__ void sq8_chunk(const float *xq, const float *sc, const float *mnv, int e,
                                          uint32_t w, float *acc) {
  const float4 s = *reinterpret_cast<const float4 *>(sc + e);
  float4 mn = make_float4(0.f, 0.f, 0.f, 0.f);
  if (kIP) mn = *reinterpret_cast<const float4 *>(mnv + e);
  const float4 x = sq8_qterm4<kIP, kCodes>(xq, s, mn, e);
  acc[0] = sq8_term<kIP>(x.x, s.x, mn.x, static_cast<float>(w & 0xffu), acc[0]);
  acc[1] = sq8_term<kIP>(x.y, s.y, mn.y, static_cast<float>((w >> 8) & 0xffu), acc[1]);
  acc[2] = sq8_term<kIP>(x.z, s.z, mn.z, static_cast<float>((w >> 16) & 0xffu), acc[2]);
  acc[3] = sq8_term<kIP>(x.w, s.w, mn.w, static_cast<float>(w >> 24), acc[3]);
}

#ifndef ALAYA_PAIR_LOOPS
#define ALAYA_PAIR_LOOPS 1
#endif
#ifndef ALAYA_SQ8_DW
#define ALAYA_SQ8_DW 48
#endif
template <int kOrder, int kFull>
constexpr int sq8_rows_per_group() {
  return kFull <= 0 ? 1 : (ALAYA_SQ8_DW / kFull >= 4 ? 4 : (ALAYA_SQ8_DW / kFull < 1 ? 1 : ALAYA_SQ8_DW / kFull));
}

template <int kOrder, int kFull>
struct Sq8Pass {
  static constexpr int P = kOrder == 2 ? 32 : 16;
  static constexpr int LPR = P / 4;
  static constexpr int G = 64 / LPR;
  static constexpr int kR = sq8_rows_per_group<kOrder, kFull>();
  static constexpr int kStep = G * kR;
  uint32_t id[kR];
  bool act[kR];
  uint32_t w[kR][kFull > 0 ? kFull : 1];
};

template <int kOrder, int kFull, bool kSkip = false>
__device__ __forceinline__ void sq8_issue(const SearchParams &p, const uint32_t *ids, int n, int base,
                                          Sq8Pass<kOrder, kFull> &S) {
  static_assert(kFull > 0, "compile-time chunk count only");
  using SP = Sq8Pass<kOrder, kFull>;
  const int lane = lane_id();
  const int g = lane / SP::LPR, m = lane % SP::LPR;
  const uint32_t id0 = stand_in_row<kSkip>(ids[base]);
#pragma unroll
  for (int r = 0; r < SP::kR; ++r) {
    const int idx = base + g + SP::G * r;
// ... 703 lines not shown
```

### alayalite_amd/csrc/search_kernels.h

```cpp
#pragma once
#include <hip/hip_runtime_api.h>

#include <cstddef>
#include <cstdint>

#include "search_variants.h"

namespace alaya_amd {

struct SearchParams {
  const float *base;
  uint64_t n;
  uint32_t dim;
  uint32_t stride;
  const uint32_t *valid;
  bool ip;
  bool generic;
  const uint32_t *l0;
  uint32_t R;
  bool dedup_edges;
  const uint32_t *levels;
  const uint64_t *upper_off;
  const uint32_t *upper_edges;
  uint32_t upper_R;
  uint32_t ep;
  const uint32_t *eps;
  uint32_t n_eps;
  const float *queries;
  uint64_t nq;
  uint32_t q_stride;
  uint32_t k;
  uint32_t ef;
  uint32_t *out_ids;
  float *out_dists;
  uint32_t *out_counters;
  uint32_t fill_id;
  uint32_t *work_counter;
  uint32_t *overflow_bits;
  uint32_t *dirty_words;
  uint32_t dirty_cap;
  uint32_t wave_lds;
  uint32_t hash_log2;
  uint32_t vis_rbits;
  uint32_t vis_lbits;
  uint32_t vis_max_disp;
  uint32_t vis_limit;
  uint16_t *spill_table;
  uint32_t stab_log2;
  uint32_t stab_rbits;
  uint32_t spill_flags;
  uint64_t *stamps;
  int sq8_order;
  const uint8_t *codes;
  uint32_t code_stride;
  const float *sq_min;
  const float *sq_max;
  uint32_t help;
  uint32_t help_flags;
  uint32_t memo_off;
  uint32_t two_waves;
  uint32_t *help_stats;
  uint32_t screen;
  const uint16_t *screen_rows;
  const float *screen_err;
  const uint8_t *screen_u8;
  uint32_t *screen_stats;
  uint32_t scout;
  uint32_t *scout_stats;
  uint32_t scout_policy;
  uint32_t *scout_policy_stats;
};
constexpr uint32_t kScoutOn = 1, kScoutVerify = 2, kScoutMiss = 4;
constexpr uint32_t kScoutEarly = 1, kScoutRecheck = 2;
constexpr uint32_t kScoutSlots = 3;
constexpr uint32_t kScoutR = 32;
constexpr size_t kScoutBoardBytes = kScoutSlots * (kScoutR * 4 + 8 + 4) + 20;

struct FilterParams {
  const uint32_t *allow;
  const uint32_t *mask_of_query;
  uint32_t mask_words;
  uint32_t k;
  uint32_t result_off;
};

struct HopParams {
  uint32_t *n_through;
};

struct RerankParams {
  const uint32_t *search_ids;
  uint32_t k;
  uint32_t n_src;
  uint32_t n_take;
  uint32_t zeros;
  uint32_t fill_id;
  uint32_t *out_ids;
  float *out_dists;
};

constexpr uint32_t kVisWide = 0xffffffffu;
constexpr size_t kHelpBoardBytes = 256;
#ifndef ALAYA_HELP_DEPTH
#define ALAYA_HELP_DEPTH 1
#endif
constexpr size_t kHelpMemoSlots = ALAYA_HELP_DEPTH + 1;
constexpr uint32_t kStabBucket = 8;
inline size_t visited_table_bytes(uint32_t hash_log2, bool compact) {
  return (static_cast<size_t>(compact ? 2 : 4)) << hash_log2;
}
size_t search_wave_lds_bytes(uint32_t stride, uint32_t ef, uint32_t hash_log2, bool compact = false,
                             int sq8_order = 0);
size_t search_query_lds_bytes(uint32_t stride, int sq8_order);
__host__ __device__ inline size_t search_shared_lds_bytes(uint32_t stride, bool sq8) {
  return sq8 ? 2 * static_cast<size_t>(stride) * 4 : 0;
}
hipError_t launch_rerank(const SearchParams &p, const RerankParams &r, hipStream_t stream);
hipError_t search_occupancy(const SearchVariant &v, bool ip, int waves, size_t lds, int *blocks_per_cu);
hipError_t launch_screen_rows(const float *base, uint64_t first, uint64_t count, uint32_t stride,
                              uint16_t *out_rows, float *out_err, hipStream_t stream);
hipError_t launch_screen_rows_u8(const float *base, uint64_t first, uint64_t count, uint32_t stride,
                                 uint8_t *out_recs, hipStream_t stream);
hipError_t launch_search(const SearchVariant &v, const SearchParams &p, int grid, int waves, size_t lds,
                         hipStream_t stream);
size_t filter_result_lds_bytes(uint32_t k);
hipError_t filtered_search_occupancy(uint32_t dim, bool generic, bool ip, int waves, size_t lds, int *blocks_per_cu);
hipError_t launch_filtered_search(const SearchParams &p, const FilterParams &f, int grid, int waves, size_t lds,
                                  hipStream_t stream);
hipError_t filtered_hop_search_occupancy(uint32_t dim, bool generic, bool ip, int waves, size_t lds, int *blocks_per_cu);
hipError_t launch_filtered_hop_search(const SearchParams &p, const FilterParams &f, const HopParams &h, int grid, int waves,
                                      size_t lds, hipStream_t stream);
hipError_t filtered_sq8_search_occupancy(uint32_t dim, int sq8_order, bool ip, int waves, size_t lds,
                                         int *blocks_per_cu);
hipError_t launch_filtered_sq8_search(const SearchParams &p, const FilterParams &f, int grid, int waves, size_t lds,
                                      hipStream_t stream);
hipError_t launch_row_distances(const SearchParams &p, const uint32_t *ids, uint32_t n,
                                uint32_t nq, float *out, hipStream_t stream);

hipError_t launch_stream_read(const void *buf, uint64_t bytes, int grid, int shape, float *sink,
                              hipStream_t stream);

}
```

### alayalite_amd/csrc/search_kernels.hip

```cpp
#include <hip/hip_runtime.h>

#include <cfloat>
#include <cstdint>

#include "screen_bound.h"
#include "search_kernels.h"
#include "search_device.h"

#ifndef ALAYA_MIN_WAVES_SQ8
#define ALAYA_MIN_WAVES_SQ8 -1
#endif
#ifndef ALAYA_MIN_WAVES_NARROW
#define ALAYA_MIN_WAVES_NARROW 0
#endif
#ifndef ALAYA_MIN_WAVES_WIDE
#define ALAYA_MIN_WAVES_WIDE 0
#endif
template <int kSpace>
constexpr bool space_sq8() { return kSpace == 1 || kSpace == 2; }
template <int kSpace>
constexpr bool space_tab() { return kSpace == 2; }

template <int kChunks, int kSpace, int kMode = 0>
constexpr int search_min_waves() {
// ... 503 lines not shown
    b->state = 0u;
    b->early = 0u;
  }
}

__device__ __forceinline__ void scout_query_end(ScoutBoard *b) {
  if (lane_id() == 0) lds_store(&b->state, 0u);
  lds_order();
  scout_post(b, 0, 3, kEmpty, kEmpty, kEmpty);
}

__device__ __forceinline__ void scout_query_begin(ScoutBoard *b, uint32_t epoch) {
  lds_order();
  if (lane_id() == 0) lds_store(&b->state, epoch);
}

__device__ __forceinline__ bool scout_lookup(ScoutBoard *b, uint32_t epoch, uint32_t u, bool fresh, uint32_t slot, float *cd) {
  const int lane = lane_id();
  bool memo_ok = false;
  const uint64_t key = scout_key(epoch, u);
  uint64_t tg = 0ull;
  if (lane < static_cast<int>(kScoutSlots)) tg = lds_load(&b->tag[lane]);
  const uint64_t rows = ballot(tg == key);
  if (rows != 0ull) {
    const int row = __ffsll(static_cast<unsigned long long>(rows)) - 1;
    lds_order();
    const uint32_t mb = lds_load(&b->bound[row][lane & static_cast<int>(kScoutR - 1)]);
    lds_order();
    const uint64_t again = lds_load(&b->tag[row]);
    memo_ok = ballot(again != key || (fresh && (mb == kScoutMissing || lane >= static_cast<int>(kScoutR)))) == 0ull;
    if (memo_ok && fresh) cd[slot] = __uint_as_float(mb);
  }
  if (lane == 0) lds_store(&b->req[0], kEmpty);
  return memo_ok;
}

__device__ __forceinline__ void scout_count_screen(ScoutBoard *b, bool hit) {
  if (lane_id() == 0) {
    b->stat[0] += 1u;
    if (hit) b->stat[1] += 1u;
  }
}

__device__ __forceinline__ void scout_early_request(ScoutBoard *b, const Lds &L, const PoolState &ps, bool keep, float lb3,
                                                    uint32_t c, uint32_t pred) {
  const uint32_t kb = keep ? (lb3 > 0.f ? __float_as_uint(lb3) : 0u) : 0xffffffffu;
  uint32_t mn = min(kb, lane_xor<1>(kb));
  mn = min(mn, lane_xor<2>(mn));
  mn = min(mn, lane_xor<4>(mn));
  mn = min(mn, lane_xor<8>(mn));
  mn = min(mn, lane_xor<16>(mn));
  mn = min(read_lane(mn, 0), read_lane(mn, 32));
  if (__uint_as_float(mn) < L.pd[ps.cur]) {
    const uint32_t cand = read_lane(c, __ffsll(static_cast<unsigned long long>(ballot(kb == mn))) - 1);
    scout_post(b, 1, 2, cand, pred, kEmpty);
    if (lane_id() == 0 && (b->early & 0xffffu) != 0xffffu) b->early += 1u;
  }
}

__device__ __forceinline__ void scout_count_mismatches(ScoutBoard *b, uint32_t bad, int lane) {
  if (lane == 0 && bad != 0u) b->stat[2] += bad;
}

__device__ __forceinline__ void scout_retarget(ScoutBoard *b, bool early, uint32_t nx, uint32_t old_pred) {
  if (early && lane_id() == 0 && lds_load(&b->req[1]) == nx && (b->early >> 16) != 0xffffu) b->early += 0x10000u;
  scout_post(b, 1, 2, nx, old_pred, kEmpty);
}

__device__ __forceinline__ void scout_leave(const SearchParams &p, ScoutBoard *b, uint64_t slot) {
  const int lane = lane_id();
  if (lane == 0) lds_store(&b->state, kScoutDone);
  if (p.scout_stats != nullptr && lane == 0) {
    p.scout_stats[4 * slot] = b->stat[0];
    p.scout_stats[4 * slot + 1] = b->stat[1];
    p.scout_stats[4 * slot + 3] = b->stat[2];
  }
  if (p.scout_policy_stats != nullptr && lane == 0) {
    p.scout_policy_stats[3 * slot] = b->early & 0xffffu;
    p.scout_policy_stats[3 * slot + 1] = b->early >> 16;
  }
}

template <int kChunks>
__device__ void scout_loop(const SearchParams &p, const Lds &Ls, ScoutBoard *b, uint64_t slot) {
  uint32_t *stats = p.scout_stats != nullptr ? p.scout_stats + 4 * slot : nullptr;
  uint32_t *policy_stats = p.scout_policy_stats != nullptr ? p.scout_policy_stats + 3 * slot : nullptr;
  const int lane = lane_id();
  const int mine = screen_pass_row(lane);
  const int R = static_cast<int>(p.R);
  const uint32_t rec = screen_u8_record_bytes(p.stride);
  const bool miss = (p.scout & kScoutMiss) != 0u;
  const bool recheck = (p.scout_policy & kScoutRecheck) != 0u;
  __builtin_amdgcn_s_setprio(0);
  ScreenQuery sq{};
  uint32_t sq_epoch = 0u;
  uint32_t records = 0u, abandoned = 0u;
  for (;;) {
    const uint32_t e = read_lane(lds_load(&b->state), 0);
    if (e == kScoutDone) break;
    if (e == 0u) {
      __builtin_amdgcn_s_sleep(8);
      continue;
    }
    if (e != sq_epoch) {
      lds_order();
      sq = screen_query_codes<kChunks>(p, Ls.q);
      lds_order();
      sq_epoch = read_lane(lds_load(&b->state), 0) == e ? e : 0u;
      continue;
    }
    uint32_t rq = kEmpty;
    uint64_t tg = 0ull;
    if (lane < static_cast<int>(kScoutSlots)) {
      rq = lds_load(&b->req[lane]);
      tg = lds_load(&b->tag[lane]);
    }
    lds_order();
    if (read_lane(lds_load(&b->state), 0) != sq_epoch) continue;
    const uint32_t u = read_lane(rq, 0), c1 = read_lane(rq, 1), c2 = read_lane(rq, 2);
    const uint64_t ku = scout_key(e, u), k1 = scout_key(e, c1), k2 = scout_key(e, c2);
    tg &= ~kScoutNoMatch;
    const bool have1 = ballot(tg == k1) != 0ull, have2 = ballot(tg == k2) != 0ull;
    uint32_t node = kEmpty;
    if (!miss && c1 != kEmpty && !have1) {
      node = c1;
    } else if (c2 != kEmpty && !have2) {
      node = c2;
    }
    const uint64_t spare = ballot(lane < static_cast<int>(kScoutSlots) && tg != ku && tg != k1 && tg != k2);
    if (node == kEmpty || spare == 0ull) {
      __builtin_amdgcn_s_sleep(8);
      continue;
    }
    const int row = __ffsll(static_cast<unsigned long long>(spare)) - 1;
    const uint32_t v = adjacency_row(p, R, node);
    const int cnt = adjacency_count(R, v);
    bool want = lane < cnt;
    want = want && !sibling_visited<0>(p, Ls, 0, v, want);
    const uint64_t wm = ballot(want);
    if (recheck) {
      lds_order();
      uint32_t rq2 = kEmpty;
      if (lane < static_cast<int>(kScoutSlots)) rq2 = lds_load(&b->req[lane]);
      lds_order();
      const uint32_t e2 = read_lane(lds_load(&b->state), 0);
      if (e2 != e || (read_lane(rq2, 1) != node && read_lane(rq2, 2) != node)) {
        ++abandoned;
        continue;
      }
    }
    if (lane == 0) lds_store(&b->tag[row], 0ull);
    lds_order();
    uint32_t lb_bits = kScoutMissing;
    if (wm != 0ull) {
      const uint32_t v0 = read_lane(v, __ffsll(static_cast<unsigned long long>(wm)) - 1);
      const uint32_t id = want ? v : v0;
      const uint32_t idm = static_cast<uint32_t>(__builtin_amdgcn_ds_bpermute(mine << 2, static_cast<int>(id)));
      const uint8_t *rp = p.screen_u8 + static_cast<uint64_t>(idm) * rec;
      const float4 head = *reinterpret_cast<const float4 *>(rp);
      const uint2 sums = *reinterpret_cast<const uint2 *>(rp + screen_u8_sums_offset(p.stride));
      const uint32_t ac = screen_dots_pass<kChunks>(p, sq.codes, id, NoHook());
      const float lb = screen_int_bound(p.stride, sq.err, sq.lo, sq.scale, sq.a1, sq.a2, head.x, head.y, head.z, sums.x,
                                        sums.y, ac);
      if ((wm >> mine) & 1ull) lb_bits = __float_as_uint(lb);
      records += static_cast<uint32_t>(__popcll(wm));
    }
    if (lane < 32 && mine < R) lds_store(&b->bound[row][mine], lb_bits);
    lds_order();
    if (lane == 0) lds_store(&b->tag[row], scout_key(e, node) | (miss ? kScoutNoMatch : 0ull));
  }
  if (stats != nullptr && lane == 0) stats[2] = records;
  if (policy_stats != nullptr && lane == 0) policy_stats[2] = abandoned;
}

__device__ __forceinline__ void screen_stats_out(const SearchParams &p, uint64_t slot, uint32_t n_screened,
                                                 uint32_t n_screened_out, int lane) {
  if (p.screen_stats != nullptr && lane == 0) {
    p.screen_stats[2 * slot] = n_screened;
    p.screen_stats[2 * slot + 1] = n_screened_out;
  }
}

template <bool kIP, int kChunks, int kMode, int kSpace = 0>
__global__ void __launch_bounds__(256)
    __attribute__((amdgpu_waves_per_eu(search_min_waves<kChunks, kSpace, kMode>() ? search_min_waves<kChunks, kSpace, kMode>() : 1,
                                       8))) hnsw_search_kernel(SearchParams p) {
  extern __shared__ __attribute__((aligned(16))) unsigned char smem[];
  constexpr bool kStamp = (kMode & kModeStamp) != 0;
  constexpr bool kCheck = (kMode & kModeCheck) != 0;
  constexpr bool kHelp = (kMode & kModeHelp) != 0;
  constexpr int kRows = (kMode & kModeTwoWaves) != 0 ? 1 : 0;
  constexpr bool kScreen = (kMode & kModeScreen) != 0;
  static_assert(!kScreen || (kSpace == 0 && !kIP && !kHelp && kChunks >= 16 && kChunks % 2 == 0), "screen: wide f32 L2 rows");
  constexpr int kScreenRows = (kMode & kModeTwoWaves) != 0 ? 2 : 4;
  constexpr int kScreenRowsU8 = 4;
  uint32_t n_screened = 0, n_screened_out = 0;
  const int lane = lane_id();
  const int wave = static_cast<int>(threadIdx.x >> 6);
  constexpr bool kScout = kScreen && (kMode & kModeTwoWaves) != 0;
  const bool scouting = kScout && p.scout != 0u;
  const bool early = scouting && p.screen == 3 && (p.scout_policy & kScoutEarly) != 0u;
  const int W = static_cast<int>(blockDim.x >> 6) >> (scouting ? 1 : 0);
  ScoutBoard *sboard = nullptr;
  if constexpr (kScout) {
    if (scouting) {
      sboard = scout_board(p, smem, W, wave < W ? wave : wave - W);
      if (wave < W) scout_board_init(sboard);
      __syncthreads();
      if (wave >= W) {
        scout_loop<kChunks>(p, carve_lds<kSpace>(p, smem, wave - W), sboard,
                            static_cast<uint64_t>(blockIdx.x) * W + (wave - W));
        return;
      }
      __builtin_amdgcn_s_setprio(2);
    }
  }
  const Lds L = carve_lds<kSpace>(p, smem, wave);
  fill_shared<kSpace>(p, L);
  HelpBoard *board = kHelp ? help_board(p, smem, W) : nullptr;
  HelpMine mine;
  if constexpr (kHelp) {
    if constexpr (ALAYA_HELP_PRIO > 0) __builtin_amdgcn_s_setprio(ALAYA_HELP_PRIO);
    if (threadIdx.x == 0) help_board_init(board);
    __syncthreads();
    for (int s = 0; s < kHelpSlots; ++s) mine.node[s] = kEmpty, mine.seq[s] = 0u;
    mine.next_seq = 0u;
    mine.memo_wave = -1;
  }
  const uint64_t bit_words = (p.n + 31) / 32;
  const uint64_t slot = static_cast<uint64_t>(blockIdx.x) * W + wave;
  uint32_t *slot_bits = p.overflow_bits + slot * bit_words;
  uint32_t *slot_dirty = p.dirty_words + slot * p.dirty_cap;
  uint16_t *slot_stab = (space_tab<kSpace>() && p.spill_table) ? p.spill_table + (slot << p.stab_log2) : nullptr;

  bool first_round = true;
  for (;;) {
    uint32_t qi = 0;
    if (kHelp && first_round) {
      qi = static_cast<uint32_t>(wave) * gridDim.x + blockIdx.x;
    } else {
      if (lane == 0) qi = atomicAdd(p.work_counter, 1u);
      qi = read_lane(qi, 0) + (kHelp ? static_cast<uint32_t>(W) * gridDim.x : 0u);
    }
    first_round = false;
    if (qi >= p.nq) break;
    if constexpr (kHelp) mine_reset(board, wave, mine);
    if constexpr (kScout) {
      if (scouting) scout_query_end(sboard);
    }

    uint64_t st[8] = {0, 0, 0, 0, 0, 0, 0, 0};
    uint64_t t_prev = kStamp ? __builtin_readcyclecounter() : 0;
    const uint64_t t_begin = t_prev;
    auto stamp = [&](int slot) {
      if constexpr (kStamp) {
        const uint64_t now = __builtin_readcyclecounter();
        st[slot] += now - t_prev;
        t_prev = now;
      }
    };
    Visited vs;
    PoolState ps;
    uint32_t n_dist = 0, n_expand = 0, n_dist_up = 0, n_hops_up = 0;
    query_begin<kIP, kChunks, kSpace, kRows>(p, L, qi, slot_bits, slot_dirty, slot_stab, vs, ps, n_dist_up, n_hops_up);
    ScreenQuery sq{};
    if constexpr (kScreen) {
      if (p.screen == 3) sq = screen_query_codes<kChunks>(p, L.q);
    }
    if constexpr (kScout) {
      if (scouting) scout_query_begin(sboard, qi + 1u);
    }

    stamp(0);
    uint32_t pred = kEmpty, pred_v = kEmpty;
    constexpr bool kSpillPrefetch = kSpace != 0;
    constexpr bool kRegMerge = kSpace == 0 && kChunks > 0 && kChunks <= 8;
    uint32_t pre_u = kEmpty;
    uint64_t pre_lo = 0ull, pre_hi = 0ull;
    while (ps.cur < ps.size) {
      uint32_t c1 = kEmpty, c2 = kEmpty;
      const uint32_t u = pool_pop<kHelp || kScout>(ps, L, &c1, &c2);
      ++n_expand;
      if constexpr (kScout) {
        if (scouting && ps.size == ps.ef) scout_post(sboard, 0, 3, u, c1, c2);
      }
      uint32_t look = 0u;
      if constexpr (kHelp) {
        if (mine.memo_wave < 0 && (n_expand & 3u) == 1u) {
          const uint32_t hw = help_word(board);
          if ((hw >> 8) != 0u) mine.memo_wave = static_cast<int>(hw >> 8) - 1;
        }
        if (mine.memo_wave >= 0) {
#pragma unroll
          for (int hs = 0; hs < kHelpSlots; ++hs)
            if (mine.node[hs] == u) look = (mine.seq[hs] << 2) | static_cast<uint32_t>(hs);
          mine_request(board, wave, mine, u, c1, c2);
        }
      }
#ifndef ALAYA_FINE_STAMPS
      if (kStamp && vs.spilled) st[5]++;
#endif
      stamp(1);
      uint32_t v;
      if (u == pred) {
        v = pred_v;
#ifndef ALAYA_FINE_STAMPS
        if (kStamp) st[7]++;
#endif
      } else {
        v = adjacency_row(p, static_cast<int>(p.R), u);
      }
      const uint64_t endm = ballot(lane < static_cast<int>(p.R) && v == kEmpty);
      const int cnt = endm ? __ffsll(static_cast<unsigned long long>(endm)) - 1 : static_cast<int>(p.R);
      bool act = lane < cnt;
#ifdef ALAYA_FINE_STAMPS
      stamp(2);
#endif
      if (p.dedup_edges) {
        for (int j = 0; j < cnt; ++j) {
          const uint32_t vj = read_lane(v, j);
          if (j < lane && vj == v) act = false;
        }
      }
      if (!vs.spilled && vs.count + 64 > vs.limit) spill_begin<space_tab<kSpace>()>(vs);
      if constexpr (kCheck && space_tab<kSpace>()) {
        if (u == pre_u && vs.spilled && vs.stab != nullptr) {
          stab_order();
          uint32_t home, code;
          stab_key(vs, v, home, code);
          uint64_t lo2 = 0ull, hi2 = 0ull;
          if (act) stab_load(vs, home, lo2, hi2);
          if (ballot(act && (lo2 != pre_lo || hi2 != pre_hi))) n_hops_up |= 0x40000000u;
        }
      }
      const bool fresh = visit<space_tab<kSpace>()>(vs, v, act, kSpillPrefetch && u == pre_u, pre_lo, pre_hi);
      if constexpr (kSpillPrefetch) {
        __builtin_amdgcn_sched_barrier(0);
        asm volatile("" ::: "memory");
      }
      pre_u = kEmpty;
      pre_lo = pre_hi = 0ull;
      const uint64_t fm = ballot(fresh);
      const int nf = __popcll(fm);
      pred = ps.cur < ps.size ? (L.pi[ps.cur] & kIdMask) : kEmpty;
      if (pred != kEmpty) pred_v = adjacency_row(p, static_cast<int>(p.R), pred, pred_v);
#ifdef ALAYA_FINE_STAMPS
      stamp(5);
#else
      stamp(2);
#endif
      if (nf == 0) continue;
      const uint32_t slot = __popcll(fm & ((1ull << lane) - 1ull));
      if (fresh) L.cid[slot] = v;
      bool memo_ok = false;
      if constexpr (kScout) {
        if (scouting && ps.size == ps.ef && p.screen == 3) memo_ok = scout_lookup(sboard, qi + 1u, u, fresh, slot, L.cd);
      }
      const uint32_t *dist_ids = L.cid;
      bool compute = true;
      if constexpr (kHelp) {
        if (look != 0u) {
          const uint32_t seq = look >> 2;
          const int hs = static_cast<int>(look & 3u);
          const uint64_t *memo = help_memo<kSpace>(p, smem, mine.memo_wave) +
                                 (static_cast<uint32_t>(wave) * kHelpSlots + hs) * p.R;
          uint64_t e = 0ull;
          if (fresh) e = __hip_atomic_load(memo + lane, __ATOMIC_RELAXED, __HIP_MEMORY_SCOPE_WORKGROUP);
          const bool got = fresh && static_cast<uint32_t>(e >> 32) == seq;
          help_retire(board, wave, hs, seq);
          uint32_t *ids2 = reinterpret_cast<uint32_t *>(L.sd);
          if (fresh) {
            ids2[slot] = got ? kEmpty : v;
            if (got) L.cd[slot] = __uint_as_float(static_cast<uint32_t>(e));
          }
          dist_ids = ids2;
          const uint32_t n_got = __popcll(ballot(got));
          help_count(board, wave, n_got, static_cast<uint32_t>(nf), lane);
          compute = n_got < static_cast<uint32_t>(nf);
        }
      }
      wave_sync();
      auto second_level_prefetch = [&]() {
        if constexpr (kSpillPrefetch) {
          if (vs.spilled && pred != kEmpty && !(p.spill_flags & 1u)) {
            if (p.spill_flags & 4u) __builtin_amdgcn_s_waitcnt(0);
            spill_prefetch(vs, pred_v, lane < static_cast<int>(p.R), pre_lo, pre_hi);
            pre_u = pred;
          }
        }
      };
      int nd = nf;
      if constexpr (kScreen) {
        if (ps.size == ps.ef) {
          const float tau = L.pd[ps.size - 1];
          const bool in = lane < nf;
          const uint32_t c = in ? L.cid[lane] : 0u;
          float e_row = 0.f;
          float lb3 = 0.f;
          if (p.screen == 3 && kScout && memo_ok) {
            lb3 = L.cd[lane];
            scout_count_screen(sboard, true);
            if (p.scout & kScoutVerify) {
              const uint8_t *rp = p.screen_u8 + static_cast<uint64_t>(c) * screen_u8_record_bytes(p.stride);
              const float4 head = *reinterpret_cast<const float4 *>(rp);
              const uint2 sums = *reinterpret_cast<const uint2 *>(rp + screen_u8_sums_offset(p.stride));
              wave_sync();
              screen_dots_int<kChunks>(p, sq.codes, L.cid, nf, reinterpret_cast<uint32_t *>(L.cd), NoHook());
              const float own = screen_int_bound(p.stride, sq.err, sq.lo, sq.scale, sq.a1, sq.a2, head.x, head.y, head.z,
                                                 sums.x, sums.y, __float_as_uint(L.cd[lane]));
              const uint32_t bad = static_cast<uint32_t>(__popcll(ballot(in && __float_as_uint(own) != __float_as_uint(lb3))));
              scout_count_mismatches(sboard, bad, lane);
            }
          } else if (p.screen == 3) {
            if constexpr (kScout) {
              if (scouting) scout_count_screen(sboard, false);
            }
            const uint8_t *rp = p.screen_u8 + static_cast<uint64_t>(c) * screen_u8_record_bytes(p.stride);
            const float4 head = *reinterpret_cast<const float4 *>(rp);
            const uint2 sums = *reinterpret_cast<const uint2 *>(rp + screen_u8_sums_offset(p.stride));
            screen_dots_int<kChunks>(p, sq.codes, L.cid, nf, reinterpret_cast<uint32_t *>(L.cd), second_level_prefetch);
            lb3 = screen_int_bound(p.stride, sq.err, sq.lo, sq.scale, sq.a1, sq.a2, head.x, head.y, head.z, sums.x, sums.y,
                                   __float_as_uint(L.cd[lane]));
          } else if (p.screen == 2) {
            if (in) e_row = *reinterpret_cast<const float *>(p.screen_u8 + static_cast<uint64_t>(c) * screen_u8_record_bytes(p.stride));
            screen_distances_u8<kChunks, kScreenRowsU8>(p, L.q, L.cid, nf, L.cd, second_level_prefetch);
          } else {
            if (in) e_row = p.screen_err[c];
            screen_distances<kChunks, kScreenRows>(p, L.q, L.cid, nf, L.cd, second_level_prefetch);
          }
          bool keep = false;
          if (in) {
            const float lb = p.screen == 3 ? lb3 : screen_lower_bound(L.cd[lane], e_row, p.dim);
            keep = !(lb > 0.f && lb >= tau);
          }
          const uint64_t km = ballot(keep);
          nd = __popcll(km);
          n_screened += static_cast<uint32_t>(nf);
          n_screened_out += static_cast<uint32_t>(nf - nd);
          if constexpr (kScout) {
            if (early && nd > 0 && ps.cur < ps.size) scout_early_request(sboard, L, ps, keep, lb3, c, pred);
          }
          if (keep) L.cid[__popcll(km & ((1ull << lane) - 1ull))] = c;
          wave_sync();
          if (nd == 0) {
            stamp(3);
            n_dist += nf;
            continue;
          }
        }
      }
      if constexpr (kScreen) {
        constexpr int kFull = RowPass<kChunks, kRows>::kR;
        if (nd <= 8) {
          space_distances<kIP, kChunks, kSpace, false, 1>(p, L, L.cid, nd, L.cd);
        } else if (kFull > 2 && nd <= 16) {
          space_distances<kIP, kChunks, kSpace, false, 2>(p, L, L.cid, nd, L.cd);
        } else {
          space_distances<kIP, kChunks, kSpace, false, kRows>(p, L, L.cid, nd, L.cd);
        }
      } else if (!kHelp || compute) {
        space_distances<kIP, kChunks, kSpace, kHelp, kRows>(p, L, dist_ids, nf, L.cd, second_level_prefetch);
      } else {
        second_level_prefetch();
      }
      stamp(3);
      n_dist += nf;
      const bool has = lane < nd;
      const uint32_t cid = has ? L.cid[lane] : 0u;
      const float cd = has ? L.cd[lane] : 0.f;
      wave_sync();
      pool_merge<kRegMerge>(ps, L, has, cid, cd, [&](uint32_t nx) {
        if (nx != pred) {
          const uint32_t old_pred = pred;
          (void)old_pred;
          pred = nx;
          if (lane < static_cast<int>(p.R)) pred_v = p.l0[static_cast<uint64_t>(nx) * p.R + lane];
          if constexpr (kHelp) {
            if (mine.memo_wave >= 0) mine_request(board, wave, mine, kEmpty, nx, old_pred);
          }
          if constexpr (kScout) {
            if (scouting && ps.size == ps.ef) scout_retarget(sboard, early, nx, old_pred);
          }
        }
      }
#ifdef ALAYA_FINE_STAMPS
      , [&]() { stamp(7); }
#endif
      );
      stamp(4);
    }

    query_end(p, L, ps, qi, n_dist, n_expand, n_dist_up, n_hops_up);
    visit_end(vs);
    if constexpr (kStamp) {
      st[6] = __builtin_readcyclecounter() - t_begin;
      if (lane < 8) p.stamps[static_cast<uint64_t>(qi) * 8 + lane] = st[lane & 7];
    }
    wave_sync();
  }
  if constexpr (kHelp) {
    help_siblings<kIP, kChunks, kSpace>(p, smem, L, board, wave, W);
    help_stats_out(p, board, wave, slot, lane);
  }
  if constexpr (kScout) {
    if (scouting) scout_leave(p, sboard, slot);
  }
  if constexpr (kScreen) screen_stats_out(p, slot, n_screened, n_screened_out, lane);
}

__global__ void __launch_bounds__(256) screen_rows_kernel(const float *base, uint64_t first, uint64_t count,
                                                          uint32_t stride, uint16_t *out_rows, float *out_err) {
  const int lane = lane_id();
  const uint64_t waves = static_cast<uint64_t>(gridDim.x) * (blockDim.x >> 6);
  for (uint64_t r = static_cast<uint64_t>(blockIdx.x) * (blockDim.x >> 6) + (threadIdx.x >> 6); r < count; r += waves) {
    const float *row = base + (first + r) * stride;
    uint16_t *dst = out_rows + (first + r) * stride;
    float sum = 0.f;
    bool bad = false;
    for (uint32_t e = 2 * lane; e < stride; e += 128) {
      const float2 x = *reinterpret_cast<const float2 *>(row + e);
      const _Float16 h0 = static_cast<_Float16>(x.x), h1 = static_cast<_Float16>(x.y);
      const float y0 = static_cast<float>(h0), y1 = static_cast<float>(h1);
      bad = bad || !(fabsf(y0) <= 65504.f) || !(fabsf(y1) <= 65504.f) || !(fabsf(x.x) <= FLT_MAX) ||
            !(fabsf(x.y) <= FLT_MAX);
      const float d0 = x.x - y0, d1 = x.y - y1;
      sum = fmaf(d0, d0, sum);
      sum = fmaf(d1, d1, sum);
      const half2_t h = {h0, h1};
      *reinterpret_cast<uint32_t *>(dst + e) = __builtin_bit_cast(uint32_t, h);
    }
    sum += lane_xor<1>(sum);
    sum += lane_xor<2>(sum);
    sum += lane_xor<4>(sum);
    sum += lane_xor<8>(sum);
    sum += lane_xor<16>(sum);
    sum = read_lane(sum, 0) + read_lane(sum, 32);
    const bool any_bad = ballot(bad) != 0ull;
    if (lane == 0) {
      float err = sqrtf(sum * (1.0f + screen_gamma(stride))) * (1.0f + 1.9073486328125e-6f) + 8.8817841970012523e-16f;
      if (any_bad || !(err <= kScreenHuge)) err = __builtin_inff();
      out_err[first + r] = err;
    }
  }
}

__global__ void __launch_bounds__(256) screen_rows_u8_kernel(const float *base, uint64_t first, uint64_t count,
                                                             uint32_t stride, uint8_t *out_recs) {
  const int lane = lane_id();
  const uint32_t rec = screen_u8_record_bytes(stride);
  const uint64_t waves = static_cast<uint64_t>(gridDim.x) * (blockDim.x >> 6);
  for (uint64_t r = static_cast<uint64_t>(blockIdx.x) * (blockDim.x >> 6) + (threadIdx.x >> 6); r < count; r += waves) {
    const float *row = base + (first + r) * stride;
    uint8_t *dst = out_recs + (first + r) * rec;
    float lo = FLT_MAX, hi = -FLT_MAX;
    bool bad = false;
    for (uint32_t e = 4 * lane; e < stride; e += 256) {
      const float4 x = *reinterpret_cast<const float4 *>(row + e);
      bad = bad || !screen_finite(x.x) || !screen_finite(x.y) || !screen_finite(x.z) || !screen_finite(x.w);
      lo = fminf(fminf(lo, x.x), fminf(fminf(x.y, x.z), x.w));
      hi = fmaxf(fmaxf(hi, x.x), fmaxf(fmaxf(x.y, x.z), x.w));
    }
    lo = fminf(lo, lane_xor<1>(lo)); hi = fmaxf(hi, lane_xor<1>(hi));
    lo = fminf(lo, lane_xor<2>(lo)); hi = fmaxf(hi, lane_xor<2>(hi));
    lo = fminf(lo, lane_xor<4>(lo)); hi = fmaxf(hi, lane_xor<4>(hi));
    lo = fminf(lo, lane_xor<8>(lo)); hi = fmaxf(hi, lane_xor<8>(hi));
    lo = fminf(lo, lane_xor<16>(lo)); hi = fmaxf(hi, lane_xor<16>(hi));
    lo = fminf(read_lane(lo, 0), read_lane(lo, 32));
    hi = fmaxf(read_lane(hi, 0), read_lane(hi, 32));
    float scale = screen_u8_scale(lo, hi);
    if (ballot(bad) != 0ull || !screen_finite(scale)) {
      bad = true;
      lo = scale = 0.f;
    }
    float sum = 0.f;
    uint32_t s1 = 0u, s2 = 0u;
    for (uint32_t e = 4 * lane; e < stride; e += 256) {
      const float4 x = *reinterpret_cast<const float4 *>(row + e);
      const uint32_t c0 = screen_u8_code(x.x, lo, scale), c1 = screen_u8_code(x.y, lo, scale);
      const uint32_t c2 = screen_u8_code(x.z, lo, scale), c3 = screen_u8_code(x.w, lo, scale);
      s1 += (c0 + c1) + (c2 + c3);
      s2 += (c0 * c0 + c1 * c1) + (c2 * c2 + c3 * c3);
      const float d0 = x.x - screen_u8_value(c0, lo, scale), d1 = x.y - screen_u8_value(c1, lo, scale);
      const float d2 = x.z - screen_u8_value(c2, lo, scale), d3 = x.w - screen_u8_value(c3, lo, scale);
      if (!bad) {
        sum = fmaf(d0, d0, sum);
        sum = fmaf(d1, d1, sum);
        sum = fmaf(d2, d2, sum);
        sum = fmaf(d3, d3, sum);
      }
      *reinterpret_cast<uint32_t *>(dst + kScreenU8Header + e) = c0 | (c1 << 8) | (c2 << 16) | (c3 << 24);
    }
    sum += lane_xor<1>(sum);
    sum += lane_xor<2>(sum);
    sum += lane_xor<4>(sum);
    sum += lane_xor<8>(sum);
    sum += lane_xor<16>(sum);
    sum = read_lane(sum, 0) + read_lane(sum, 32);
    s1 += lane_xor<1>(s1); s2 += lane_xor<1>(s2);
    s1 += lane_xor<2>(s1); s2 += lane_xor<2>(s2);
    s1 += lane_xor<4>(s1); s2 += lane_xor<4>(s2);
    s1 += lane_xor<8>(s1); s2 += lane_xor<8>(s2);
    s1 += lane_xor<16>(s1); s2 += lane_xor<16>(s2);
    s1 = read_lane(s1, 0) + read_lane(s1, 32);
    s2 = read_lane(s2, 0) + read_lane(s2, 32);
    if (lane == 0) {
      *reinterpret_cast<float4 *>(dst) = make_float4(screen_u8_err(sum, stride, bad), lo, scale, 0.f);
      *reinterpret_cast<uint2 *>(dst + screen_u8_sums_offset(stride)) = make_uint2(s1, s2);
    }
  }
}

template <bool kIP>
__global__ void __launch_bounds__(64) row_distance_kernel(SearchParams p, const uint32_t *ids,
                                                          uint32_t n, float *out) {
  extern __shared__ __attribute__((aligned(16))) unsigned char smem[];
  float *q = reinterpret_cast<float *>(smem);
  uint32_t *lid = reinterpret_cast<uint32_t *>(smem + static_cast<size_t>(p.stride) * 4);
  float *ld = reinterpret_cast<float *>(lid + 64);
  const int lane = lane_id();
  const float *qsrc = p.queries + static_cast<uint64_t>(blockIdx.y) * p.q_stride;
  for (uint32_t e = lane; e < p.stride; e += 64) q[e] = e < p.dim ? qsrc[e] : 0.f;
  wave_sync();
  for (uint32_t b = blockIdx.x * 64; b < n; b += gridDim.x * 64) {
    const uint32_t cnt = min(64u, n - b);
    if (static_cast<uint32_t>(lane) < cnt) lid[lane] = ids[b + lane];
    wave_sync();
    for (uint32_t c = 0; c < cnt; c += 8)
      row_distances<kIP, 0>(p, q, lid + c, min(8u, cnt - c), ld + c);
    if (static_cast<uint32_t>(lane) < cnt)
      out[static_cast<uint64_t>(blockIdx.y) * n + b + lane] = ld[lane];
    wave_sync();
  }
}


template <bool kIP>
__global__ void __launch_bounds__(64) rerank_kernel(SearchParams p, RerankParams rp) {
  extern __shared__ __attribute__((aligned(16))) unsigned char smem[];
  float *q = reinterpret_cast<float *>(smem);
  uint32_t *cid = reinterpret_cast<uint32_t *>(smem + static_cast<size_t>(p.stride) * 4);
  const uint32_t cap = max(rp.k, rp.n_src) + 1;
  float *cd = reinterpret_cast<float *>(cid + cap);
  uint32_t *cm = reinterpret_cast<uint32_t *>(cd + cap);
  const int lane = lane_id();
  const uint32_t taken = rp.n_take;
  const uint32_t zeros = rp.zeros;
  const uint32_t c = taken + (zeros ? 1u : 0u);
  const float fill_d = rp.fill_id == kEmpty ? FLT_MAX : 0.f;
  for (uint64_t qi = blockIdx.x; qi < p.nq; qi += gridDim.x) {
    const float *qsrc = p.queries + qi * p.q_stride;
    for (uint32_t e = lane; e < p.stride; e += 64) q[e] = e < p.dim ? qsrc[e] : 0.f;
    uint32_t nv = 0;
    for (uint32_t b = 0; b < c; b += 64) {
      const uint32_t i = b + lane;
      uint32_t id = 0, m = 0;
      if (i < c) {
        id = i < taken ? rp.search_ids[qi * rp.n_src + i] : 0u;
        m = i < taken ? 1u : zeros;
        if (id == kEmpty) {
          id = 0u;
          m = 0u;
        }
        cid[i] = id;
        cm[i] = m;
      }
      for (int off = 32; off > 0; off >>= 1) m += __shfl_xor(m, off);
      nv += m;
    }
    wave_sync();
    row_distances<kIP, 0>(p, q, cid, static_cast<int>(c), cd);
    for (uint32_t i = lane; i < c; i += 64) {
      const float di = cd[i];
      const uint32_t ii = cid[i];
      uint32_t rank = 0;
      for (uint32_t j = 0; j < c; ++j) {
        const float dj = cd[j];
        const uint32_t ij = cid[j];
        const bool less = dj < di || (dj == di && ij < ii);
        const bool tie_before = dj == di && ij == ii && j < i;
        if (less || tie_before) rank += cm[j];
      }
      for (uint32_t m = 0; m < cm[i] && rank + m < rp.k; ++m) {
        rp.out_ids[qi * rp.k + rank + m] = ii;
        if (rp.out_dists) rp.out_dists[qi * rp.k + rank + m] = di;
      }
    }
    for (uint32_t i = nv + lane; i < rp.k; i += 64) {
      rp.out_ids[qi * rp.k + i] = rp.fill_id;
// ... 119 lines not shown
      pool_merge<kRegMerge>(ps, L, has, cid, cd, [&](uint32_t nx) {
        if (nx != pred) {
          pred = nx;
          pred_v = adjacency_row(p, static_cast<int>(p.R), nx, pred_v);
        }
      });
      result_offer(rs, Lr, has && (((aw & vw) >> (cid & 31)) & 1u) != 0u, cid, cd);
    }

    query_end(p, Lr, rs, qi, n_dist, n_expand, n_dist_up, n_hops_up);
    visit_end(vs);
    wave_sync();
  }
}
}

hipError_t launch_stream_read(const void *buf, uint64_t bytes, int grid, int shape, float *sink,
                              hipStream_t stream) {
  const float4 *p = static_cast<const float4 *>(buf);
  if (shape == 1) {
    hipLaunchKernelGGL(stream_read_kernel<1>, dim3(grid), dim3(256), 0, stream, p, bytes / 16, sink);
  } else if (shape == 2) {
    hipLaunchKernelGGL(stream_read_kernel<2>, dim3(grid), dim3(256), 0, stream, p, bytes / 16, sink);
  } else {
    hipLaunchKernelGGL(stream_read_kernel<0>, dim3(grid), dim3(256), 0, stream, p, bytes / 16, sink);
  }
  return hipGetLastError();
}

size_t search_query_lds_bytes(uint32_t stride, int sq8_order) {
  return sq8_order == 2 && sq8_query_codes<2>() ? (static_cast<size_t>(stride) + 15) / 16 * 16
                                                : static_cast<size_t>(stride) * 4;
}

size_t search_wave_lds_bytes(uint32_t stride, uint32_t ef, uint32_t hash_log2, bool compact, int sq8_order) {
  return search_query_lds_bytes(stride, sq8_order) + 3 * 64 * 4 + 2 * (((ef + 1) * 4 + 15) / 16 * 16) +
         visited_table_bytes(hash_log2, compact);
}

hipError_t launch_rerank(const SearchParams &p, const RerankParams &r, hipStream_t stream) {
  const size_t lds = static_cast<size_t>(p.stride) * 4 + 3 * (static_cast<size_t>(std::max(r.k, r.n_src)) + 1) * 4 + 64;
  const int grid = static_cast<int>(std::min<uint64_t>(p.nq, 4096));
  if (p.ip) {
    hipLaunchKernelGGL(rerank_kernel<true>, dim3(grid), dim3(64), lds, stream, p, r);
  } else {
    hipLaunchKernelGGL(rerank_kernel<false>, dim3(grid), dim3(64), lds, stream, p, r);
  }
  return hipGetLastError();
}

template <bool kIP, int kChunks, int kMode, int kSpace>
static const void *kernel_ptr() {
  return reinterpret_cast<const void *>(&hnsw_search_kernel<kIP, kChunks, kMode, kSpace>);
}

struct SearchKernels {
  const void *ip, *l2;
};
#define ALAYA_IP_both(S, C, M) kernel_ptr<true, C, M, S>()
#define ALAYA_IP_l2(S, C, M) nullptr
#define ALAYA_KERNEL_ROW(S, C, M, METRICS) {ALAYA_IP_##METRICS(S, C, M), kernel_ptr<false, C, M, S>()},
static const SearchKernels kSearchKernels[] = {ALAYA_SEARCH_VARIANTS(ALAYA_KERNEL_ROW)};
#undef ALAYA_KERNEL_ROW
static_assert(sizeof(kSearchKernels) / sizeof(kSearchKernels[0]) == kNumSearchVariants, "one kernel row per variant");

static const void *search_kernel_symbol(const SearchVariant &v, bool ip) {
  const SearchKernels &k = kSearchKernels[&v - kSearchVariants];
  return ip ? k.ip : k.l2;
}

hipError_t launch_screen_rows(const float *base, uint64_t first, uint64_t count, uint32_t stride,
                              uint16_t *out_rows, float *out_err, hipStream_t stream) {
  if (count == 0) return hipSuccess;
  const int grid = static_cast<int>(std::min<uint64_t>((count + 3) / 4, 16384));
  hipLaunchKernelGGL(screen_rows_kernel, dim3(grid), dim3(256), 0, stream, base, first, count, stride, out_rows,
                     out_err);
  return hipGetLastError();
}

hipError_t launch_screen_rows_u8(const float *base, uint64_t first, uint64_t count, uint32_t stride,
                                 uint8_t *out_recs, hipStream_t stream) {
  if (count == 0) return hipSuccess;
  const int grid = static_cast<int>(std::min<uint64_t>((count + 3) / 4, 16384));
  hipLaunchKernelGGL(screen_rows_u8_kernel, dim3(grid), dim3(256), 0, stream, base, first, count, stride, out_recs);
  return hipGetLastError();
}

hipError_t launch_search(const SearchVariant &v, const SearchParams &p, int grid, int waves, size_t lds,
                         hipStream_t stream) {
  SearchParams arg = p;
  void *args[] = {&arg};
  return hipLaunchKernel(search_kernel_symbol(v, p.ip), dim3(grid), dim3(64 * waves), args, lds, stream);
}

hipError_t launch_row_distances(const SearchParams &p, const uint32_t *ids, uint32_t n,
                                uint32_t nq, float *out, hipStream_t stream) {
  const size_t lds = static_cast<size_t>(p.stride) * 4 + 128 * 4;
  const int gx = static_cast<int>(std::min<uint32_t>((n + 63) / 64, 1024u));
  if (p.ip) {
    hipLaunchKernelGGL(row_distance_kernel<true>, dim3(gx, nq), dim3(64), lds, stream, p, ids, n, out);
  } else {
    hipLaunchKernelGGL(row_distance_kernel<false>, dim3(gx, nq), dim3(64), lds, stream, p, ids, n, out);
  }
  return hipGetLastError();
}

hipError_t search_occupancy(const SearchVariant &v, bool ip, int waves, size_t lds, int *blocks_per_cu) {
  return hipOccupancyMaxActiveBlocksPerMultiprocessor(blocks_per_cu, search_kernel_symbol(v, ip), 64 * waves, lds);
}

template <int... kChunks>
static const void *filtered_symbol_of(int chunks, bool ip) {
  const void *sym = nullptr;
  ((chunks == kChunks ? (sym = ip ? reinterpret_cast<const void *>(&filtered_search_kernel<true, kChunks>)
                                  : reinterpret_cast<const void *>(&filtered_search_kernel<false, kChunks>),
                         0)
                      : 0),
   ...);
  return sym;
}

static const void *filtered_kernel_symbol(uint32_t dim, bool generic, bool ip) {
  const void *sym = filtered_symbol_of<4, 8, 16, 24, 30, 32>(search_chunks(dim, generic), ip);
  return sym != nullptr ? sym : filtered_symbol_of<0>(0, ip);
}

size_t filter_result_lds_bytes(uint32_t k) { return 2 * ((static_cast<size_t>(k + 1) * 4 + 15) / 16 * 16); }

hipError_t launch_filtered_search(const SearchParams &p, const FilterParams &f, int grid, int waves, size_t lds,
                                  hipStream_t stream) {
  SearchParams arg = p;
  FilterParams farg = f;
  void *args[] = {&arg, &farg};
  return hipLaunchKernel(filtered_kernel_symbol(p.dim, p.generic, p.ip), dim3(grid), dim3(64 * waves), args, lds, stream);
}

hipError_t filtered_search_occupancy(uint32_t dim, bool generic, bool ip, int waves, size_t lds, int *blocks_per_cu) {
  return hipOccupancyMaxActiveBlocksPerMultiprocessor(blocks_per_cu, filtered_kernel_symbol(dim, generic, ip), 64 * waves,
                                                      lds);
}

namespace {
__device__ __forceinline__ void candidate_offer(const SearchParams &p, PoolState &rs, const Lds &Lr, bool allowed, uint32_t id,
                                                float d) {
  const bool full = rs.size == rs.ef;
  const float worst = full ? Lr.pd[rs.size - 1] : 0.f;
  bool ok = allowed && !(full && d >= worst);
  if (ballot(ok) == 0ull) return;
  if (p.valid != nullptr && ok) ok = ((p.valid[id >> 5] >> (id & 31)) & 1u) != 0u;
  pool_merge(rs, Lr, ok, id, d);
}

template <bool kIP, int kChunks, int kSpace>
__global__ void __launch_bounds__(256)
    __attribute__((amdgpu_waves_per_eu(search_min_waves<kChunks, kSpace, 0>() ? search_min_waves<kChunks, kSpace, 0>() : 1, 8)))
    filtered_sq8_search_kernel(SearchParams p, FilterParams f) {
  static_assert(space_sq8<kSpace>(), "SQ8 codes");
  extern __shared__ __attribute__((aligned(16))) unsigned char smem[];
  constexpr bool kTab = space_tab<kSpace>();
  const int lane = lane_id();
  const int wave = static_cast<int>(threadIdx.x >> 6);
  const int W = static_cast<int>(blockDim.x >> 6);
  const Lds L = carve_lds<kSpace>(p, smem, wave);
  fill_shared<kSpace>(p, L);
  const Lds Lr = result_lds(L, f);
  const uint64_t bit_words = (p.n + 31) / 32;
  const uint64_t slot = static_cast<uint64_t>(blockIdx.x) * W + wave;
// ... 337 lines not shown
```

### include/alaya_hip.h

```cpp
#ifndef ALAYA_HIP_H_
#define ALAYA_HIP_H_

#include <stddef.h>
#include <stdint.h>

#ifdef __cplusplus
extern "C" {
#endif

#define ALAYA_OK 0
#define ALAYA_ERR_ARG 1
#define ALAYA_ERR_RUNTIME 2
#define ALAYA_ERR_DEVICE 3

#define ALAYA_METRIC_L2 0
#define ALAYA_METRIC_IP 1
#define ALAYA_METRIC_COS 2
#define ALAYA_DIST_GENERIC 0x100

typedef struct alaya_index alaya_index;
typedef struct alaya_graph alaya_graph;

const char *alaya_last_error(void);
const char *alaya_build_info(void);
// ... 34 lines not shown
                                    void *stream);
int alaya_index_filtered_search(alaya_index *ix, const float *queries, uint64_t nq, uint32_t k, uint32_t ef,
                                const uint32_t *allow_words, uint32_t n_masks, const uint32_t *mask_of_query,
                                uint32_t *ids, float *dists, uint32_t *counters);
int alaya_index_filtered_search_device(alaya_index *ix, const float *d_queries, uint64_t nq, uint32_t k, uint32_t ef,
                                       const uint32_t *d_allow_words, uint32_t n_masks,
                                       const uint32_t *d_mask_of_query, uint32_t *d_ids, float *d_dists,
                                       uint32_t *d_counters, void *stream);
int alaya_index_filtered_search_hop(alaya_index *ix, const float *queries, uint64_t nq, uint32_t k, uint32_t ef,
                                    const uint32_t *allow_words, uint32_t n_masks, const uint32_t *mask_of_query,
                                    uint32_t *ids, float *dists, uint32_t *counters, uint32_t *n_through);
int alaya_index_filtered_search_hop_device(alaya_index *ix, const float *d_queries, uint64_t nq, uint32_t k, uint32_t ef,
                                           const uint32_t *d_allow_words, uint32_t n_masks,
                                           const uint32_t *d_mask_of_query, uint32_t *d_ids, float *d_dists,
                                           uint32_t *d_counters, uint32_t *d_n_through, void *stream);
int alaya_index_filtered_search_sq8(alaya_index *ix, const float *queries, const float *rerank_queries, uint64_t nq,
                                    uint32_t k, uint32_t ef, uint32_t pool, const uint32_t *allow_words,
                                    uint32_t n_masks, const uint32_t *mask_of_query, uint32_t *ids, float *dists,
                                    uint32_t *counters);
int alaya_index_filtered_search_sq8_device(alaya_index *ix, const float *d_queries, const float *d_rerank_queries,
                                           uint64_t nq, uint32_t k, uint32_t ef, uint32_t pool,
                                           const uint32_t *d_allow_words, uint32_t n_masks,
                                           const uint32_t *d_mask_of_query, uint32_t *d_ids, float *d_dists,
                                           uint32_t *d_counters, void *stream);
int alaya_index_build_graph(alaya_index *ix, uint32_t R, uint32_t ef_construction, uint64_t seed,
                            uint32_t batch_div, uint32_t max_batch, uint32_t refine, alaya_graph **out,
                            uint64_t *stats);
int alaya_index_extend_graph(alaya_index *ix, const float *rows, uint64_t count, uint32_t ef_construction,
                             uint64_t seed, uint32_t batch_div, uint32_t max_batch, uint32_t refine,
                             alaya_graph **out, uint64_t *stats);
int alaya_index_read_sq8(alaya_index *ix, uint64_t first, uint64_t count, uint8_t *codes);
int alaya_build_batches(const uint32_t *levels, uint64_t n, uint64_t start, uint32_t ep, uint32_t batch_div,
                        uint32_t max_batch, uint64_t *ends, uint64_t *n_batches);
int alaya_index_reserve(alaya_index *ix, uint64_t capacity);
int alaya_index_write_rows(alaya_index *ix, uint64_t first, const float *rows, uint64_t count);
int alaya_index_write_edges(alaya_index *ix, const uint32_t *ids, const uint32_t *edges, uint64_t count);
int alaya_index_set_valid(alaya_index *ix, uint64_t id, int valid);
int alaya_index_enable_updates(alaya_index *ix, const alaya_graph *g, const float *rows, uint64_t n,
                               uint64_t capacity, const uint8_t *valid_bitmap);
int alaya_index_insert(alaya_index *ix, const float *search_query, const float *row, uint32_t ef,
                       uint64_t *new_id);
int alaya_index_remove(alaya_index *ix, uint64_t id);
int alaya_index_export_graph(alaya_index *ix, alaya_graph **out);
int alaya_index_export_rows(alaya_index *ix, float *rows, uint8_t *valid_bitmap, uint64_t *n);
int alaya_index_distances(alaya_index *ix, const float *queries, uint64_t nq, const uint32_t *ids,
                          uint32_t n, float *out);
int alaya_index_profile_search(alaya_index *ix, const float *queries, uint64_t nq, uint32_t k,
                               uint32_t ef, int space, uint32_t *ids, uint32_t *counters, uint64_t *stamps);
int alaya_sq8_train(const float *data, uint64_t n, uint32_t dim, float *min_v, float *max_v);
int alaya_sq8_encode(const float *data, uint64_t n, uint32_t dim, const float *min_v,
                     const float *max_v, uint8_t *codes, uint32_t num_threads);
int alaya_index_set_sq8(alaya_index *ix, const uint8_t *codes, uint64_t n, uint32_t dim,
                        const float *min_v, const float *max_v, int order);
int alaya_index_batch_search_sq8(alaya_index *ix, const float *queries, const float *rerank_queries,
                                 uint64_t nq, uint32_t k, uint32_t ef, int rerank, uint32_t *ids,
                                 float *dists, uint32_t *counters);
int alaya_index_batch_search_sq8_device(alaya_index *ix, const float *d_queries, const float *d_rerank_queries,
                                        uint64_t nq, uint32_t k, uint32_t ef, int rerank, uint32_t *d_ids,
                                        float *d_dists, uint32_t *d_counters, void *stream);
int alaya_index_shard_search_sq8_device(alaya_index *ix, const float *d_queries, const float *d_rerank_queries,
                                        uint64_t nq, uint32_t k, uint32_t ef, int holds_row0, uint32_t *d_ids,
                                        float *d_dists, uint32_t *d_counters, void *stream);
int alaya_index_flat_search(alaya_index *ix, const float *queries, uint64_t nq, uint32_t k,
                            uint32_t *ids, float *dists, uint32_t *n_recomputed);
int alaya_index_flat_search_device(alaya_index *ix, const float *d_queries, uint64_t nq, uint32_t k,
                                   uint32_t *d_ids, float *d_dists, uint32_t *d_flags, void *stream);
int alaya_index_flat_last_contraction(const alaya_index *ix, int *contraction);
int alaya_index_flat_search_filtered(alaya_index *ix, const float *queries, uint64_t nq, uint32_t k,
                                     const uint32_t *allow_words, uint32_t n_masks, const uint32_t *mask_of_query,
                                     uint32_t *ids, float *dists);
int alaya_index_flat_search_filtered_device(alaya_index *ix, const float *d_queries, uint64_t nq, uint32_t k,
                                            const uint32_t *d_allow_words, uint32_t n_masks,
                                            const uint32_t *d_mask_of_query, uint32_t *d_ids, float *d_dists,
                                            void *stream);
int alaya_index_flat_filtered_last(const alaya_index *ix, uint64_t *out);
int alaya_flat_filtered_plan(uint64_t n_allowed, uint64_t nq, uint32_t k, uint32_t stride, uint32_t cus,
                             uint64_t *out);
int alaya_index_set_hash_log2(alaya_index *ix, uint32_t log2_slots);
int alaya_index_set_visited_mode(alaya_index *ix, int mode);
int alaya_index_set_helpers(alaya_index *ix, int mode);
int alaya_index_help_stats(alaya_index *ix, uint64_t *memo_dists, uint64_t *memo_expansions,
                           uint64_t *helper_rows);
int alaya_index_screen_stats(alaya_index *ix, uint64_t *screened, uint64_t *screened_out);
int alaya_screen_lower_bound(const float *d_tilde, const float *e_row, uint64_t n, uint32_t dim, float *out);
int alaya_screen_u8_quantize(const float *rows, uint64_t n, uint32_t dim, uint8_t *codes, float *header,
                             float *values);
int alaya_screen_int_bound(const float *queries, const float *rows, uint64_t n, uint32_t dim, float *d_in,
                           float *e_sum, float *bound, uint32_t *sums);
int alaya_flat_ip_slack(int contraction, uint32_t k_acc, const float *q_norm2, const int *q_exp, uint64_t n,
                        float b_max, int base_exp, float *out);
int alaya_flat_ip_proven(const float *kth_d, const float *cutoff, const float *slack, uint64_t n, uint8_t *out);
int alaya_search_variant(uint32_t dim, int ip, int sq8_order, int generic, uint32_t wanted_mode, int *space,
                         uint32_t *chunks, uint32_t *mode, uint32_t *has_mode);
int alaya_search_variant_at(uint32_t index, int *space, uint32_t *chunks, uint32_t *mode, int *l2_only,
                            uint32_t *count);
int alaya_index_last_launch(const alaya_index *ix, uint32_t *workgroups, uint32_t *waves_per_group);
int alaya_index_last_plan(const alaya_index *ix, uint32_t *lds_bytes, uint32_t *hash_log2, uint32_t *compact,
                          uint32_t *groups_per_cu, uint32_t *scout);
int alaya_index_scout_stats(alaya_index *ix, uint64_t *expansions, uint64_t *hits, uint64_t *records,
                            uint64_t *mismatches);
int alaya_index_scout_policy_stats(alaya_index *ix, uint32_t *policy, uint64_t *early_posts, uint64_t *confirmed,
                                   uint64_t *abandoned);
int alaya_index_info(const alaya_index *ix, uint64_t *n, uint32_t *dim, uint32_t *stride,
                     int *metric, uint64_t *device_bytes);

#ifdef __cplusplus
}
#endif
#endif
```

Before: 352,100.

## Add two-stage nibble screening mode for graph search candidates

Adds a screen format 4 that splits the 8-bit screening codes into a high-nibble plane and a low-nibble plane. Search first computes a cheap 4-bit lower bound from the high plane and reads the low plane only for candidates that survive, which reduces bytes read per screened candidate. The mode needs an extra screening copy in device memory, a per-search stats buffer and memset, and adds branches to the search kernel. It is enabled only through ALAYA_SEARCH_SCREEN=4, so the default path is unchanged unless screen_default selects it.

New measurement: 348,300. 0.989x the previous value.

```diff
diff --git a/alayalite_amd/csrc/capi.cpp b/alayalite_amd/csrc/capi.cpp
--- a/alayalite_amd/csrc/capi.cpp
+++ b/alayalite_amd/csrc/capi.cpp
@@ -139,10 +139,12 @@
     bool ready = false;
     bool failed = false;
   };
-  ScreenCopy screen_copy[2];
+  ScreenCopy screen_copy[3];
   uint32_t screen_format = 0;
   DevBuf screen_stats;
   uint64_t screen_stats_slots = 0;
+  DevBuf nibble_stats;
+  uint64_t nibble_stats_slots = 0;
   uint32_t last_grid = 0, last_waves = 0;
   uint32_t last_lds = 0, last_hash_log2 = 0, last_compact = 0, last_per_cu = 0, last_scout = 0;
   DevBuf scout_stats;
@@ -487,7 +489,7 @@
   p.scout = 0u;
   p.scout_policy = 0u;
   const uint32_t scout = scout_requested(ix->dim);
-  if (scout != 0u && p.screen == 3u && !p.ip && !p.two_waves && !p.help && plan.W == 1 && ix->R <= kScoutR &&
+  if (scout != 0u && (p.screen == 3u || p.screen == 4u) && !p.ip && !p.two_waves && !p.help && plan.W == 1 && ix->R <= kScoutR &&
       (plan.variant->mode & ~kModeScreen) == 0 && search_has_two_waves(ix->dim, p.sq8_order, ix->generic) &&
       !helpers_requested(ix, p, nq, cus)) {
     SearchRequest r2 = r;
@@ -557,6 +559,7 @@
   ix->scout_stats_slots = p.scout ? searchers : 0;
   ix->help_stats_slots = p.help ? searchers : 0;
   ix->screen_stats_slots = p.screen ? searchers : 0;
+  ix->nibble_stats_slots = p.screen == 4u ? searchers : 0;
   ix->work.reserve(4);
   p.work_counter = ix->work.as<uint32_t>();
   hip_check(hipMemsetAsync(p.work_counter, 0, 4, stream), "hipMemsetAsync");
@@ -577,7 +580,10 @@
   set_search_space(ix, p, sq8, ef);
   if (const char *e = std::getenv("ALAYA_HELP_FLAGS")) p.help_flags = static_cast<uint32_t>(std::strtoul(e, nullptr, 10));
   const SearchPlan plan = plan_search(ix, p, search_request(ix, p, nq, ef, stream), nq, ef, stream);
-  if (p.screen >= 2) {
+  if (p.screen == 4) {
+    p.screen_u8 = ix->screen_copy[2].rows.as<uint8_t>();
+    p.screen_lo = ix->screen_copy[2].err.as<uint8_t>();
+  } else if (p.screen >= 2) {
     p.screen_u8 = ix->screen_copy[1].rows.as<uint8_t>();
   } else if (p.screen) {
     p.screen_rows = ix->screen_copy[0].rows.as<uint16_t>();
@@ -600,6 +606,11 @@
   if (p.screen) {
     ix->screen_stats.reserve(searchers * 8);
     p.screen_stats = ix->screen_stats.as<uint32_t>();
+  }
+  if (p.screen == 4) {
+    ix->nibble_stats.reserve(searchers * 16);
+    p.nibble_stats = ix->nibble_stats.as<uint32_t>();
+    hip_check(hipMemsetAsync(p.nibble_stats, 0, searchers * 16, stream), "hipMemsetAsync");
   }
   record_launch(ix, p, plan.grid, wg_waves, plan.lds, plan.per_cu, searchers, stream);
   hip_check(alaya_amd::launch_search(*plan.variant, p, plan.grid, wg_waves, plan.lds, stream), "search launch");
@@ -664,6 +675,12 @@
 
 void screen_fill(alaya_index *ix, uint32_t format, uint64_t first, uint64_t count, hipStream_t stream) {
   alaya_index::ScreenCopy &c = ix->screen_copy[format - 1];
+  if (format == 3) {
+    hip_check(alaya_amd::launch_screen_rows_nib(ix->base.as<float>(), first, count, ix->stride, c.rows.as<uint8_t>(),
+                                                c.err.as<uint8_t>(), stream),
+              "screening copy");
+    return;
+  }
   hip_check(format == 2 ? alaya_amd::launch_screen_rows_u8(ix->base.as<float>(), first, count, ix->stride,
                                                            c.rows.as<uint8_t>(), stream)
                         : alaya_amd::launch_screen_rows(ix->base.as<float>(), first, count, ix->stride,
@@ -677,9 +694,10 @@
   const char *e = std::getenv("ALAYA_SEARCH_SCREEN");
   const int asked = e && e[0] ? std::atoi(e) : -1;
   const uint32_t format =
-      asked < 0 ? screen_default(ix->dim) : (asked == 0 ? 0u : (asked == 9 ? 3u : (asked == 8 ? 2u : 1u)));
+      asked < 0 ? screen_default(ix->dim)
+                : (asked == 0 ? 0u : (asked == 9 ? 3u : (asked == 8 ? 2u : (asked == 4 ? 4u : 1u))));
   if (format == 0) return false;
-  const uint32_t copy = format == 3 ? 2u : format;
+  const uint32_t copy = format == 4 ? 3u : (format == 3 ? 2u : format);
   alaya_index::ScreenCopy &c = ix->screen_copy[copy - 1];
   if (c.failed) return false;
   if (!c.ready) {
@@ -689,7 +707,10 @@
         c.rows.release();
         c.err.release();
         c.cap = 0;
-        if (copy == 2) {
+        if (copy == 3) {
+          c.rows.reserve(rows * alaya_amd::screen_nib_record_bytes(ix->stride));
+          c.err.reserve(rows * alaya_amd::screen_nib_record_bytes(ix->stride));
+        } else if (copy == 2) {
           c.rows.reserve(rows * alaya_amd::screen_u8_record_bytes(ix->stride));
         } else {
           c.rows.reserve(rows * ix->stride * 2);
@@ -723,6 +744,7 @@
   }
   ix->screen_format = 0;
   ix->screen_stats_slots = 0;
+  ix->nibble_stats_slots = 0;
 }
 
 void ensure_norms(alaya_index *ix, hipStream_t stream) {
@@ -1323,7 +1345,7 @@
   ix->n = std::max(ix->n, first + count);
   ix->norms_ready = false;
   ix->tiles_ready = false;
-  for (uint32_t format = 1; format <= 2; ++format) {
+  for (uint32_t format = 1; format <= 3; ++format) {
     alaya_index::ScreenCopy &c = ix->screen_copy[format - 1];
     if (!c.ready) continue;
     if (first + count <= c.cap) {
@@ -2737,6 +2759,99 @@
   });
 }
 
+namespace {
+void screen_nib_quantize_one(const float *x, uint32_t dim, uint8_t *high, uint8_t *low) {
+  using namespace alaya_amd;
+  const uint32_t rec = screen_nib_record_bytes(dim);
+  std::vector<uint8_t> c(dim);
+  float head[4];
+  screen_u8_quantize_one(x, dim, c.data(), head, nullptr);
+  bool bad = false;
+  float mn = FLT_MAX, mx = -FLT_MAX;
+  for (uint32_t j = 0; j < dim; ++j) {
+    bad = bad || !screen_finite(x[j]);
+    mn = fminf(mn, x[j]);
+    mx = fmaxf(mx, x[j]);
+  }
+  bad = bad || !screen_finite(screen_u8_scale(mn, mx));
+  const float lo4 = screen_nib_lo4(head[1], head[2]), scale4 = screen_nib_scale4(head[2]);
+  std::memset(high, 0, rec);
+  std::memset(low, 0, rec);
+  uint32_t c1 = 0, c2 = 0, h1 = 0, h2 = 0;
+  float sum4 = 0.f;
+  bool bad4 = bad || !screen_finite(lo4) || !screen_finite(scale4);
+  for (uint32_t j = 0; j < dim; ++j) {
+    const uint32_t cj = c[j], h = cj >> 4, l = cj & 15u;
+    const float d = x[j] - screen_u8_value(h, lo4, scale4);
+    if (!bad4) sum4 = fmaf(d, d, sum4);
+    c1 += cj; c2 += cj * cj;
+    h1 += h; h2 += h * h;
+    high[kScreenU8Header + screen_nib_byte(j)] |= static_cast<uint8_t>(h << screen_nib_shift(j));
+    low[kScreenU8Header + screen_nib_byte(j)] |= static_cast<uint8_t>(l << screen_nib_shift(j));
+  }
+  const float head4[4] = {screen_u8_err(sum4, dim, bad4), lo4, scale4, 0.f};
+  const uint32_t sums4[2] = {h1, h2}, sums8[2] = {c1, c2};
+  std::memcpy(high, head4, sizeof(head4));
+  std::memcpy(high + screen_nib_sums_offset(dim), sums4, sizeof(sums4));
+  std::memcpy(low, head, sizeof(head));
+  std::memcpy(low + screen_nib_sums_offset(dim), sums8, sizeof(sums8));
+}
+}
+
+int alaya_screen_nibble_record_bytes(uint32_t dim) { return static_cast<int>(alaya_amd::screen_nib_record_bytes(dim)); }
+
+int alaya_screen_nibble_quantize(const float *rows, uint64_t n, uint32_t dim, uint8_t *high, uint8_t *low) {
+  return guarded([&] {
+    if (dim == 0 || dim > 4096 || dim % 16u != 0) throw ArgError("dim must be a multiple of 16 in 16 .. 4096");
+    if (n && (!rows || !high || !low)) throw ArgError("invalid arguments");
+    const uint64_t rec = alaya_amd::screen_nib_record_bytes(dim);
+    for (uint64_t r = 0; r < n; ++r) screen_nib_quantize_one(rows + r * dim, dim, high + r * rec, low + r * rec);
+  });
+}
+
+int alaya_screen_nibble_bound(const float *queries, const float *rows, uint64_t n, uint32_t dim, float *bound4,
+                              float *bound8, uint32_t *sums) {
+  return guarded([&] {
+    using namespace alaya_amd;
+    if (dim == 0 || dim > 4096 || dim % 16u != 0) throw ArgError("dim must be a multiple of 16 in 16 .. 4096");
+    if (n && (!queries || !rows || !bound4 || !bound8 || !sums)) throw ArgError("invalid arguments");
+    const uint32_t rec = screen_nib_record_bytes(dim);
+    std::vector<uint8_t> a(dim), high(rec), low(rec);
+    for (uint64_t i = 0; i < n; ++i) {
+      float qh[4];
+      screen_u8_quantize_one(queries + i * dim, dim, a.data(), qh, nullptr);
+      screen_nib_quantize_one(rows + i * dim, dim, high.data(), low.data());
+      uint32_t a1 = 0, a2 = 0, ah = 0, al = 0;
+      for (uint32_t piece = 0; piece < dim / 16u; ++piece) {
+        uint32_t qc[4], w[2], v[2];
+        for (uint32_t k = 0; k < 4; ++k) {
+          const uint8_t *ak = a.data() + 16u * piece + 4u * k;
+          qc[k] = ak[0] | (static_cast<uint32_t>(ak[1]) << 8) | (static_cast<uint32_t>(ak[2]) << 16) |
+                  (static_cast<uint32_t>(ak[3]) << 24);
+          for (uint32_t b = 0; b < 4; ++b) {
+            a1 += ak[b];
+            a2 += static_cast<uint32_t>(ak[b]) * ak[b];
+          }
+        }
+        std::memcpy(w, high.data() + kScreenU8Header + 8u * piece, 8);
+        std::memcpy(v, low.data() + kScreenU8Header + 8u * piece, 8);
+        ah += screen_nib_piece_dot(qc, w[0], w[1]);
+        al += screen_nib_piece_dot(qc, v[0], v[1]);
+      }
+      float h4[4], h8[4];
+      uint32_t s4[2], s8[2];
+      std::memcpy(h4, high.data(), sizeof(h4));
+      std::memcpy(h8, low.data(), sizeof(h8));
+      std::memcpy(s4, high.data() + screen_nib_sums_offset(dim), sizeof(s4));
+      std::memcpy(s8, low.data() + screen_nib_sums_offset(dim), sizeof(s8));
+      bound4[i] = screen_int_bound(dim, qh[0], qh[1], qh[2], a1, a2, h4[0], h4[1], h4[2], s4[0], s4[1], ah);
+      bound8[i] = screen_int_bound(dim, qh[0], qh[1], qh[2], a1, a2, h8[0], h8[1], h8[2], s8[0], s8[1], 16u * ah + al);
+      uint32_t *s = sums + 4 * i;
+      s[0] = ah; s[1] = al; s[2] = s4[0]; s[3] = s4[1];
+    }
+  });
+}
+
 int alaya_flat_ip_slack(int contraction, uint32_t k_acc, const float *q_norm2, const int *q_exp, uint64_t n,
                         float b_max, int base_exp, float *out) {
   return guarded([&] {
@@ -2791,6 +2906,18 @@
   });
 }
 
+int alaya_index_nibble_stats(alaya_index *ix, uint64_t *stage1_out, uint64_t *stage2, uint64_t *low_searcher,
+                             uint64_t *low_scout) {
+  return guarded_scratch(ix, [&] {
+    if (!ix) throw ArgError("null index");
+    const std::vector<uint64_t> t = searcher_stats(ix, ix->nibble_stats, ix->nibble_stats_slots, 4);
+    if (stage1_out) *stage1_out = t[0];
+    if (stage2) *stage2 = t[1];
+    if (low_searcher) *low_searcher = t[2];
+    if (low_scout) *low_scout = t[3];
+  });
+}
+
 int alaya_index_set_visited_mode(alaya_index *ix, int mode) {
   return guarded([&] {
     if (!ix) throw ArgError("null index");
diff --git a/alayalite_amd/csrc/pybind_module.cpp b/alayalite_amd/csrc/pybind_module.cpp
--- a/alayalite_amd/csrc/pybind_module.cpp
+++ b/alayalite_amd/csrc/pybind_module.cpp
@@ -152,6 +152,11 @@
     uint64_t a = 0, b = 0;
     check(alaya_index_screen_stats(ix_, &a, &b));
     return py::make_tuple(a, b);
+  }
+  py::tuple nibble_stats() {
+    uint64_t a = 0, b = 0, c = 0, d = 0;
+    check(alaya_index_nibble_stats(ix_, &a, &b, &c, &d));
+    return py::make_tuple(a, b, c, d);
   }
   py::tuple scout_stats() {
     uint64_t e = 0, h = 0, r = 0, m = 0;
@@ -1203,6 +1208,7 @@
       .def("last_launch", &PyIndexInterface::last_launch)
       .def("help_stats", &PyIndexInterface::help_stats)
       .def("screen_stats", &PyIndexInterface::screen_stats)
+      .def("nibble_stats", &PyIndexInterface::nibble_stats)
       .def("scout_stats", &PyIndexInterface::scout_stats)
       .def("scout_policy_stats", &PyIndexInterface::scout_policy_stats)
       .def("last_plan", &PyIndexInterface::last_plan)
@@ -1249,6 +1255,7 @@
       .def("last_launch", &DeviceIndex::last_launch)
       .def("help_stats", &DeviceIndex::help_stats)
       .def("screen_stats", &DeviceIndex::screen_stats)
+      .def("nibble_stats", &DeviceIndex::nibble_stats)
       .def("scout_stats", &DeviceIndex::scout_stats)
       .def("scout_policy_stats", &DeviceIndex::scout_policy_stats)
       .def("last_plan", &DeviceIndex::last_plan)
@@ -1317,6 +1324,26 @@
                                  bound.mutable_data(), sums.mutable_data()));
     return py::make_tuple(d_in, e_sum, bound, sums);
   });
+  m.def("screen_nibble_record_bytes", [](uint32_t dim) { return alaya_screen_nibble_record_bytes(dim); });
+  m.def("screen_nibble_quantize", [](F32Array rows) {
+    if (rows.ndim() != 2) throw std::invalid_argument("rows must be 2-D");
+    const int rec = alaya_screen_nibble_record_bytes(static_cast<uint32_t>(rows.shape(1)));
+    py::array_t<uint8_t> high({rows.shape(0), static_cast<py::ssize_t>(rec)});
+    py::array_t<uint8_t> low({rows.shape(0), static_cast<py::ssize_t>(rec)});
+    check(alaya_screen_nibble_quantize(rows.data(), static_cast<uint64_t>(rows.shape(0)),
+                                       static_cast<uint32_t>(rows.shape(1)), high.mutable_data(), low.mutable_data()));
+    return py::make_tuple(high, low);
+  });
+  m.def("screen_nibble_bound", [](F32Array queries, F32Array rows) {
+    if (rows.ndim() != 2 || queries.ndim() != 2 || rows.shape(0) != queries.shape(0) || rows.shape(1) != queries.shape(1))
+      throw std::invalid_argument("queries and rows must be 2-D of one shape");
+    py::array_t<float> bound4(rows.shape(0)), bound8(rows.shape(0));
+    py::array_t<uint32_t> sums({rows.shape(0), static_cast<py::ssize_t>(4)});
+    check(alaya_screen_nibble_bound(queries.data(), rows.data(), static_cast<uint64_t>(rows.shape(0)),
+                                    static_cast<uint32_t>(rows.shape(1)), bound4.mutable_data(), bound8.mutable_data(),
+                                    sums.mutable_data()));
+    return py::make_tuple(bound4, bound8, sums);
+  });
   m.def("flat_filtered_plan", [](uint64_t n_allowed, uint64_t nq, uint32_t k, uint32_t stride, uint32_t cus) {
     uint64_t o[5] = {0, 0, 0, 0, 0};
     check(alaya_flat_filtered_plan(n_allowed, nq, k, stride, cus, o));
diff --git a/alayalite_amd/csrc/screen_bound.h b/alayalite_amd/csrc/screen_bound.h
--- a/alayalite_amd/csrc/screen_bound.h
+++ b/alayalite_amd/csrc/screen_bound.h
@@ -81,4 +81,23 @@
                             screen_int_err(e_row, lo, s, e_q, qlo, qs), n);
 }
 
+ALAYA_HD inline uint32_t screen_nib_record_bytes(uint32_t stride) {
+  return (kScreenU8Header + stride / 2u + 8u + 63u) & ~63u;
 }
+ALAYA_HD inline uint32_t screen_nib_sums_offset(uint32_t stride) { return kScreenU8Header + stride / 2u; }
+ALAYA_HD inline float screen_nib_scale4(float scale) { return 16.0f * scale; }
+ALAYA_HD inline float screen_nib_lo4(float lo, float scale) { return fmaf(7.5f, scale, lo); }
+
+ALAYA_HD inline uint32_t screen_nib_byte(uint32_t j) { return 8u * (j >> 4) + 4u * ((j >> 3) & 1u) + (j & 3u); }
+ALAYA_HD inline uint32_t screen_nib_shift(uint32_t j) { return 4u * ((j >> 2) & 1u); }
+
+ALAYA_HD inline uint32_t screen_nib_dot4(uint32_t a, uint32_t b) {
+  return (a & 0xffu) * (b & 0xffu) + ((a >> 8) & 0xffu) * ((b >> 8) & 0xffu) + ((a >> 16) & 0xffu) * ((b >> 16) & 0xffu) +
+         (a >> 24) * (b >> 24);
+}
+ALAYA_HD inline uint32_t screen_nib_piece_dot(const uint32_t a[4], uint32_t w0, uint32_t w1) {
+  return screen_nib_dot4(a[0], w0 & 0x0f0f0f0fu) + screen_nib_dot4(a[1], (w0 >> 4) & 0x0f0f0f0fu) +
+         screen_nib_dot4(a[2], w1 & 0x0f0f0f0fu) + screen_nib_dot4(a[3], (w1 >> 4) & 0x0f0f0f0fu);
+}
+
+}
diff --git a/alayalite_amd/csrc/search_device.h b/alayalite_amd/csrc/search_device.h
--- a/alayalite_amd/csrc/search_device.h
+++ b/alayalite_amd/csrc/search_device.h
@@ -598,6 +598,74 @@
     screen_fold<16, 2>(acc, (lane & 16) != 0);
     const uint32_t tot = acc[0] + static_cast<uint32_t>(__builtin_amdgcn_ds_bpermute((lane ^ 32) << 2, static_cast<int>(acc[0])));
     if (lane < 32 && base + mine < n) out[base + mine] = tot;
+  }
+  wave_sync();
+}
+
+__device__ __forceinline__ int lane_id_here() {
+  int l = lane_id();
+  asm volatile("" : "+v"(l));
+  return l;
+}
+
+template <int kN>
+__device__ __forceinline__ int screen_nib_row(int lane) {
+  static_assert(kN == 8 || kN == 16 || kN == 32, "rows per pass");
+  if constexpr (kN == 32) return screen_pass_row(lane);
+  if constexpr (kN == 16) return ((lane & 1) << 3) | ((lane & 2) << 1) | ((lane & 4) >> 1) | ((lane & 8) >> 3);
+  return ((lane & 1) << 2) | (lane & 2) | ((lane & 4) >> 2);
+}
+
+template <int kChunks, int kN, typename Hook>
+__device__ __forceinline__ uint32_t screen_nib_pass(const uint8_t *plane, uint32_t rec, const uint4 qc, uint32_t id,
+                                                    Hook after_issue) {
+  constexpr int kPieces = 2 * kChunks;
+  const int lane = lane_id_here();
+  const uint32_t piece = kScreenU8Header + 8u * static_cast<uint32_t>(lane < kPieces ? lane : kPieces - 1);
+  uint2 y[kN];
+#pragma unroll
+  for (int r = 0; r < kN; ++r) {
+    const uint8_t *rp = plane + static_cast<uint64_t>(read_lane(id, r)) * rec;
+    y[r] = *reinterpret_cast<const uint2 *>(rp + piece);
+  }
+  __builtin_amdgcn_sched_barrier(0);
+  after_issue();
+  uint32_t acc[kN];
+#pragma unroll
+  for (int r = 0; r < kN; ++r) {
+    uint32_t a = __builtin_amdgcn_udot4(qc.x, y[r].x & 0x0f0f0f0fu, 0u, false);
+    a = __builtin_amdgcn_udot4(qc.y, (y[r].x >> 4) & 0x0f0f0f0fu, a, false);
+    a = __builtin_amdgcn_udot4(qc.z, y[r].y & 0x0f0f0f0fu, a, false);
+    acc[r] = __builtin_amdgcn_udot4(qc.w, (y[r].y >> 4) & 0x0f0f0f0fu, a, false);
+    if ((r & 7) == 7) __builtin_amdgcn_sched_barrier(0);
+  }
+  screen_fold<1, kN>(acc, (lane & 1) != 0);
+  screen_fold<2, kN / 2>(acc, (lane & 2) != 0);
+  screen_fold<4, kN / 4>(acc, (lane & 4) != 0);
+  if constexpr (kN >= 16) {
+    screen_fold<8, kN / 8>(acc, (lane & 8) != 0);
+  } else {
+    acc[0] += lane_xor<8>(acc[0]);
+  }
+  if constexpr (kN == 32) {
+    screen_fold<16, 2>(acc, (lane & 16) != 0);
+  } else {
+    acc[0] += lane_xor<16>(acc[0]);
+  }
+  return acc[0] + static_cast<uint32_t>(__builtin_amdgcn_ds_bpermute((lane ^ 32) << 2, static_cast<int>(acc[0])));
+}
+
+template <int kChunks, int kN, typename Hook>
+__device__ __forceinline__ void screen_dots_nib(const uint8_t *plane, uint32_t rec, const uint4 qc, const uint32_t *ids,
+                                                int n, uint32_t *out, Hook after_issue) {
+  for (int base = 0; base < n; base += kN) {
+    const int lane = lane_id_here();
+    const int mine = screen_nib_row<kN>(lane);
+    const uint32_t id = ids[base + lane < n ? base + lane : base];
+    const uint32_t tot = screen_nib_pass<kChunks, kN>(plane, rec, qc, id, [&]() {
+      if (base == 0) after_issue();
+    });
+    if (lane < kN && base + mine < n) out[base + mine] = tot;
   }
   wave_sync();
 }
diff --git a/alayalite_amd/csrc/search_kernels.h b/alayalite_amd/csrc/search_kernels.h
--- a/alayalite_amd/csrc/search_kernels.h
+++ b/alayalite_amd/csrc/search_kernels.h
@@ -69,6 +69,8 @@
   uint32_t *scout_stats;
   uint32_t scout_policy;
   uint32_t *scout_policy_stats;
+  const uint8_t *screen_lo;
+  uint32_t *nibble_stats;
 };
 constexpr uint32_t kScoutOn = 1, kScoutVerify = 2, kScoutMiss = 4;
 constexpr uint32_t kScoutEarly = 1, kScoutRecheck = 2;
@@ -121,6 +123,8 @@
                               uint16_t *out_rows, float *out_err, hipStream_t stream);
 hipError_t launch_screen_rows_u8(const float *base, uint64_t first, uint64_t count, uint32_t stride,
                                  uint8_t *out_recs, hipStream_t stream);
+hipError_t launch_screen_rows_nib(const float *base, uint64_t first, uint64_t count, uint32_t stride,
+                                  uint8_t *out_high, uint8_t *out_low, hipStream_t stream);
 hipError_t launch_search(const SearchVariant &v, const SearchParams &p, int grid, int waves, size_t lds,
                          hipStream_t stream);
 size_t filter_result_lds_bytes(uint32_t k);
diff --git a/alayalite_amd/csrc/search_kernels.hip b/alayalite_amd/csrc/search_kernels.hip
--- a/alayalite_amd/csrc/search_kernels.hip
+++ b/alayalite_amd/csrc/search_kernels.hip
@@ -609,6 +609,61 @@
 }
 
 template <int kChunks>
+__device__ __forceinline__ uint32_t scout_nibble_bounds(const SearchParams &p, const Lds &Ls, ScoutBoard *b, uint32_t e,
+                                                        const ScreenQuery &sq, uint32_t v, bool want, uint64_t wm,
+                                                        uint32_t &low_records) {
+  const int lane = lane_id();
+  const uint32_t rec = screen_nib_record_bytes(p.stride);
+  const uint32_t v0 = read_lane(v, __ffsll(static_cast<unsigned long long>(wm)) - 1);
+  const uint32_t id = want ? v : v0;
+  const uint8_t *rp = p.screen_u8 + static_cast<uint64_t>(id) * rec;
+  const float4 head = *reinterpret_cast<const float4 *>(rp);
+  const uint2 sums = *reinterpret_cast<const uint2 *>(rp + screen_nib_sums_offset(p.stride));
+  const uint32_t ahm = screen_nib_pass<kChunks, 32>(p.screen_u8, rec, sq.codes, id, NoHook());
+  const uint32_t ah = static_cast<uint32_t>(__builtin_amdgcn_ds_bpermute(screen_pass_row(lane) << 2, static_cast<int>(ahm)));
+  const float lb4 = screen_int_bound(p.stride, sq.err, sq.lo, sq.scale, sq.a1, sq.a2, head.x, head.y, head.z, sums.x,
+                                     sums.y, ah);
+  lds_order();
+  const uint32_t ts_bits = read_lane(lds_load(reinterpret_cast<const uint32_t *>(Ls.pd) + (p.ef - 1u)), 0);
+  lds_order();
+  const bool same = read_lane(lds_load(&b->state), 0) == e;
+  const float tau_s = (same && ts_bits != 0u && ts_bits < 0x7f800000u) ? __uint_as_float(ts_bits) : INFINITY;
+  const bool s1 = want && !(lb4 >= tau_s);
+  const uint64_t m1 = ballot(s1);
+  uint32_t word = __float_as_uint(lb4);
+  if (m1 != 0ull) {
+    const int n1 = __popcll(m1);
+    const uint32_t rank = static_cast<uint32_t>(__popcll(m1 & ((1ull << lane) - 1ull)));
+    const int dst = static_cast<int>(s1 ? rank : 63u) << 2;
+    uint32_t id2 = static_cast<uint32_t>(__builtin_amdgcn_ds_permute(dst, static_cast<int>(id)));
+    const uint32_t ah2 = static_cast<uint32_t>(__builtin_amdgcn_ds_permute(dst, static_cast<int>(ah)));
+    const uint32_t lb4_2 = static_cast<uint32_t>(__builtin_amdgcn_ds_permute(dst, static_cast<int>(word)));
+    id2 = lane < n1 ? id2 : read_lane(id2, 0);
+    const uint8_t *rq = p.screen_lo + static_cast<uint64_t>(id2) * rec;
+    const float4 head8 = *reinterpret_cast<const float4 *>(rq);
+    const uint2 sums8 = *reinterpret_cast<const uint2 *>(rq + screen_nib_sums_offset(p.stride));
+    uint32_t al;
+    if (n1 <= 8) {
+      const uint32_t t = screen_nib_pass<kChunks, 8>(p.screen_lo, rec, sq.codes, id2, NoHook());
+      al = static_cast<uint32_t>(__builtin_amdgcn_ds_bpermute(screen_nib_row<8>(lane_id_here()) << 2, static_cast<int>(t)));
+    } else if (n1 <= 16) {
+      const uint32_t t = screen_nib_pass<kChunks, 16>(p.screen_lo, rec, sq.codes, id2, NoHook());
+      al = static_cast<uint32_t>(__builtin_amdgcn_ds_bpermute(screen_nib_row<16>(lane_id_here()) << 2, static_cast<int>(t)));
+    } else {
+      const uint32_t t = screen_nib_pass<kChunks, 32>(p.screen_lo, rec, sq.codes, id2, NoHook());
+      al = static_cast<uint32_t>(__builtin_amdgcn_ds_bpermute(screen_nib_row<32>(lane) << 2, static_cast<int>(t)));
+    }
+    const float lb8 = screen_int_bound(p.stride, sq.err, sq.lo, sq.scale, sq.a1, sq.a2, head8.x, head8.y, head8.z,
+                                       sums8.x, sums8.y, 16u * ah2 + al);
+    const uint32_t both = max(lb4_2, __float_as_uint(lb8));
+    const uint32_t back = static_cast<uint32_t>(__builtin_amdgcn_ds_bpermute(static_cast<int>(rank) << 2, static_cast<int>(both)));
+    if (s1) word = back;
+    low_records += static_cast<uint32_t>(n1);
+  }
+  return want ? word : kScoutMissing;
+}
+
+template <int kChunks>
 __device__ void scout_loop(const SearchParams &p, const Lds &Ls, ScoutBoard *b, uint64_t slot) {
   uint32_t *stats = p.scout_stats != nullptr ? p.scout_stats + 4 * slot : nullptr;
   uint32_t *policy_stats = p.scout_policy_stats != nullptr ? p.scout_policy_stats + 3 * slot : nullptr;
@@ -616,12 +671,13 @@
   const int mine = screen_pass_row(lane);
   const int R = static_cast<int>(p.R);
   const uint32_t rec = screen_u8_record_bytes(p.stride);
+  const bool nib = p.screen == 4u;
   const bool miss = (p.scout & kScoutMiss) != 0u;
   const bool recheck = (p.scout_policy & kScoutRecheck) != 0u;
   __builtin_amdgcn_s_setprio(0);
   ScreenQuery sq{};
   uint32_t sq_epoch = 0u;
-  uint32_t records = 0u, abandoned = 0u;
+  uint32_t records = 0u, abandoned = 0u, low_records = 0u;
   for (;;) {
     const uint32_t e = read_lane(lds_load(&b->state), 0);
     if (e == kScoutDone) break;
@@ -679,7 +735,11 @@
     if (lane == 0) lds_store(&b->tag[row], 0ull);
     lds_order();
     uint32_t lb_bits = kScoutMissing;
-    if (wm != 0ull) {
+    if (nib) {
+      if (wm != 0ull) lb_bits = scout_nibble_bounds<kChunks>(p, Ls, b, e, sq, v, want, wm, low_records);
+      records += static_cast<uint32_t>(__popcll(wm));
+      if (lane < R) lds_store(&b->bound[row][lane], lb_bits);
+    } else if (wm != 0ull) {
       const uint32_t v0 = read_lane(v, __ffsll(static_cast<unsigned long long>(wm)) - 1);
       const uint32_t id = want ? v : v0;
       const uint32_t idm = static_cast<uint32_t>(__builtin_amdgcn_ds_bpermute(mine << 2, static_cast<int>(id)));
@@ -692,11 +752,12 @@
       if ((wm >> mine) & 1ull) lb_bits = __float_as_uint(lb);
       records += static_cast<uint32_t>(__popcll(wm));
     }
-    if (lane < 32 && mine < R) lds_store(&b->bound[row][mine], lb_bits);
+    if (!nib && lane < 32 && mine < R) lds_store(&b->bound[row][mine], lb_bits);
     lds_order();
     if (lane == 0) lds_store(&b->tag[row], scout_key(e, node) | (miss ? kScoutNoMatch : 0ull));
   }
   if (stats != nullptr && lane == 0) stats[2] = records;
+  if (nib && p.nibble_stats != nullptr && lane == 0) p.nibble_stats[4 * slot + 3] = low_records;
   if (policy_stats != nullptr && lane == 0) policy_stats[2] = abandoned;
 }
 
@@ -722,11 +783,12 @@
   constexpr int kScreenRows = (kMode & kModeTwoWaves) != 0 ? 2 : 4;
   constexpr int kScreenRowsU8 = 4;
   uint32_t n_screened = 0, n_screened_out = 0;
+  uint32_t n_stage1_out = 0, n_stage2 = 0, n_low = 0;
   const int lane = lane_id();
   const int wave = static_cast<int>(threadIdx.x >> 6);
   constexpr bool kScout = kScreen && (kMode & kModeTwoWaves) != 0;
   const bool scouting = kScout && p.scout != 0u;
-  const bool early = scouting && p.screen == 3 && (p.scout_policy & kScoutEarly) != 0u;
+  const bool early = scouting && p.screen >= 3 && (p.scout_policy & kScoutEarly) != 0u;
   const int W = static_cast<int>(blockDim.x >> 6) >> (scouting ? 1 : 0);
   ScoutBoard *sboard = nullptr;
   if constexpr (kScout) {
@@ -792,7 +854,7 @@
     query_begin<kIP, kChunks, kSpace, kRows>(p, L, qi, slot_bits, slot_dirty, slot_stab, vs, ps, n_dist_up, n_hops_up);
     ScreenQuery sq{};
     if constexpr (kScreen) {
-      if (p.screen == 3) sq = screen_query_codes<kChunks>(p, L.q);
+      if (p.screen >= 3) sq = screen_query_codes<kChunks>(p, L.q);
     }
     if constexpr (kScout) {
       if (scouting) scout_query_begin(sboard, qi + 1u);
@@ -881,7 +943,7 @@
       if (fresh) L.cid[slot] = v;
       bool memo_ok = false;
       if constexpr (kScout) {
-        if (scouting && ps.size == ps.ef && p.screen == 3) memo_ok = scout_lookup(sboard, qi + 1u, u, fresh, slot, L.cd);
+        if (scouting && ps.size == ps.ef && p.screen >= 3) memo_ok = scout_lookup(sboard, qi + 1u, u, fresh, slot, L.cd);
       }
       const uint32_t *dist_ids = L.cid;
       bool compute = true;
@@ -920,14 +982,37 @@
       if constexpr (kScreen) {
         if (ps.size == ps.ef) {
           const float tau = L.pd[ps.size - 1];
-          const bool in = lane < nf;
-          const uint32_t c = in ? L.cid[lane] : 0u;
+          bool in = lane < nf;
+          uint32_t c = in ? L.cid[lane] : 0u;
           float e_row = 0.f;
           float lb3 = 0.f;
-          if (p.screen == 3 && kScout && memo_ok) {
+          if (p.screen >= 3 && kScout && memo_ok) {
             lb3 = L.cd[lane];
             scout_count_screen(sboard, true);
-            if (p.scout & kScoutVerify) {
+            if ((p.scout & kScoutVerify) && p.screen == 4) {
+              const uint32_t rec4 = screen_nib_record_bytes(p.stride);
+              const uint8_t *rp = p.screen_u8 + static_cast<uint64_t>(c) * rec4;
+              const uint8_t *rq = p.screen_lo + static_cast<uint64_t>(c) * rec4;
+              const float4 head = *reinterpret_cast<const float4 *>(rp);
+              const uint2 sums = *reinterpret_cast<const uint2 *>(rp + screen_nib_sums_offset(p.stride));
+              const float4 head8 = *reinterpret_cast<const float4 *>(rq);
+              const uint2 sums8 = *reinterpret_cast<const uint2 *>(rq + screen_nib_sums_offset(p.stride));
+              wave_sync();
+              screen_dots_nib<kChunks, 32>(p.screen_u8, rec4, sq.codes, L.cid, nf, reinterpret_cast<uint32_t *>(L.cd), NoHook());
+              const uint32_t ah = __float_as_uint(L.cd[lane]);
+              wave_sync();
+              screen_dots_nib<kChunks, 32>(p.screen_lo, rec4, sq.codes, L.cid, nf, reinterpret_cast<uint32_t *>(L.cd), NoHook());
+              const uint32_t al = __float_as_uint(L.cd[lane]);
+              const float own4 = screen_int_bound(p.stride, sq.err, sq.lo, sq.scale, sq.a1, sq.a2, head.x, head.y, head.z,
+                                                  sums.x, sums.y, ah);
+              const float own8 = screen_int_bound(p.stride, sq.err, sq.lo, sq.scale, sq.a1, sq.a2, head8.x, head8.y,
+                                                  head8.z, sums8.x, sums8.y, 16u * ah + al);
+              const uint32_t mb = __float_as_uint(lb3);
+              const bool same = mb == max(__float_as_uint(own4), __float_as_uint(own8)) ||
+                                (mb == __float_as_uint(own4) && own4 >= tau);
+              scout_count_mismatches(sboard, static_cast<uint32_t>(__popcll(ballot(in && !same))), lane);
+              n_low += static_cast<uint32_t>(nf);
+            } else if (p.scout & kScoutVerify) {
               const uint8_t *rp = p.screen_u8 + static_cast<uint64_t>(c) * screen_u8_record_bytes(p.stride);
               const float4 head = *reinterpret_cast<const float4 *>(rp);
               const uint2 sums = *reinterpret_cast<const uint2 *>(rp + screen_u8_sums_offset(p.stride));
@@ -948,6 +1033,49 @@
             screen_dots_int<kChunks>(p, sq.codes, L.cid, nf, reinterpret_cast<uint32_t *>(L.cd), second_level_prefetch);
             lb3 = screen_int_bound(p.stride, sq.err, sq.lo, sq.scale, sq.a1, sq.a2, head.x, head.y, head.z, sums.x, sums.y,
                                    __float_as_uint(L.cd[lane]));
+          } else if (p.screen == 4) {
+            if constexpr (kScout) {
+              if (scouting) scout_count_screen(sboard, false);
+            }
+            const uint32_t rec4 = screen_nib_record_bytes(p.stride);
+            const uint8_t *rp = p.screen_u8 + static_cast<uint64_t>(c) * rec4;
+            const float4 head = *reinterpret_cast<const float4 *>(rp);
+            const uint2 sums = *reinterpret_cast<const uint2 *>(rp + screen_nib_sums_offset(p.stride));
+            screen_dots_nib<kChunks, 32>(p.screen_u8, rec4, sq.codes, L.cid, nf, reinterpret_cast<uint32_t *>(L.cd),
+                                         second_level_prefetch);
+            const uint32_t ah = __float_as_uint(L.cd[lane]);
+            const float lb4 = screen_int_bound(p.stride, sq.err, sq.lo, sq.scale, sq.a1, sq.a2, head.x, head.y, head.z, sums.x,
+                                               sums.y, ah);
+            const bool s1 = in && !(lb4 > 0.f && lb4 >= tau);
+            const uint64_t m1 = ballot(s1);
+            const int n1 = __popcll(m1);
+            n_stage1_out += static_cast<uint32_t>(nf - n1);
+            n_stage2 += static_cast<uint32_t>(n1);
+            n_low += static_cast<uint32_t>(n1);
+            const uint32_t rank = static_cast<uint32_t>(__popcll(m1 & ((1ull << lane) - 1ull)));
+            const int dst = static_cast<int>(s1 ? rank : 63u) << 2;
+            if (s1) L.cid[rank] = c;
+            const uint32_t ah2 = static_cast<uint32_t>(__builtin_amdgcn_ds_permute(dst, static_cast<int>(ah)));
+            const float lb4_2 = __uint_as_float(static_cast<uint32_t>(__builtin_amdgcn_ds_permute(dst, static_cast<int>(__float_as_uint(lb4)))));
+            wave_sync();
+            in = lane < n1;
+            c = in ? L.cid[lane] : 0u;
+            if (n1 > 0) {
+              const uint8_t *rq = p.screen_lo + static_cast<uint64_t>(c) * rec4;
+              const float4 head8 = *reinterpret_cast<const float4 *>(rq);
+              const uint2 sums8 = *reinterpret_cast<const uint2 *>(rq + screen_nib_sums_offset(p.stride));
+              uint32_t *al_out = reinterpret_cast<uint32_t *>(L.cd);
+              if (n1 <= 8) {
+                screen_dots_nib<kChunks, 8>(p.screen_lo, rec4, sq.codes, L.cid, n1, al_out, NoHook());
+              } else if (n1 <= 16) {
+                screen_dots_nib<kChunks, 16>(p.screen_lo, rec4, sq.codes, L.cid, n1, al_out, NoHook());
+              } else {
+                screen_dots_nib<kChunks, 32>(p.screen_lo, rec4, sq.codes, L.cid, n1, al_out, NoHook());
+              }
+              const float lb8 = screen_int_bound(p.stride, sq.err, sq.lo, sq.scale, sq.a1, sq.a2, head8.x, head8.y, head8.z,
+                                                 sums8.x, sums8.y, 16u * ah2 + __float_as_uint(L.cd[lane]));
+              lb3 = fmaxf(lb4_2, lb8);
+            }
           } else if (p.screen == 2) {
             if (in) e_row = *reinterpret_cast<const float *>(p.screen_u8 + static_cast<uint64_t>(c) * screen_u8_record_bytes(p.stride));
             screen_distances_u8<kChunks, kScreenRowsU8>(p, L.q, L.cid, nf, L.cd, second_level_prefetch);
@@ -957,7 +1085,7 @@
           }
           bool keep = false;
           if (in) {
-            const float lb = p.screen == 3 ? lb3 : screen_lower_bound(L.cd[lane], e_row, p.dim);
+            const float lb = p.screen >= 3 ? lb3 : screen_lower_bound(L.cd[lane], e_row, p.dim);
             keep = !(lb > 0.f && lb >= tau);
           }
           const uint64_t km = ballot(keep);
@@ -1032,7 +1160,14 @@
   if constexpr (kScout) {
     if (scouting) scout_leave(p, sboard, slot);
   }
-  if constexpr (kScreen) screen_stats_out(p, slot, n_screened, n_screened_out, lane);
+  if constexpr (kScreen) {
+    screen_stats_out(p, slot, n_screened, n_screened_out, lane);
+    if (p.screen == 4 && p.nibble_stats != nullptr && lane == 0) {
+      p.nibble_stats[4 * slot] = n_stage1_out;
+      p.nibble_stats[4 * slot + 1] = n_stage2;
+      p.nibble_stats[4 * slot + 2] = n_low;
+    }
+  }
 }
 
 __global__ void __launch_bounds__(256) screen_rows_kernel(const float *base, uint64_t first, uint64_t count,
@@ -1071,10 +1206,11 @@
   }
 }
 
+template <bool kNib>
 __global__ void __launch_bounds__(256) screen_rows_u8_kernel(const float *base, uint64_t first, uint64_t count,
-                                                             uint32_t stride, uint8_t *out_recs) {
+                                                             uint32_t stride, uint8_t *out_recs, uint8_t *out_low) {
   const int lane = lane_id();
-  const uint32_t rec = screen_u8_record_bytes(stride);
+  const uint32_t rec = kNib ? screen_nib_record_bytes(stride) : screen_u8_record_bytes(stride);
   const uint64_t waves = static_cast<uint64_t>(gridDim.x) * (blockDim.x >> 6);
   for (uint64_t r = static_cast<uint64_t>(blockIdx.x) * (blockDim.x >> 6) + (threadIdx.x >> 6); r < count; r += waves) {
     const float *row = base + (first + r) * stride;
@@ -1101,6 +1237,9 @@
     }
     float sum = 0.f;
     uint32_t s1 = 0u, s2 = 0u;
+    const float lo4 = screen_nib_lo4(lo, scale), scale4 = screen_nib_scale4(scale);
+    float sum4 = 0.f;
+    uint32_t h1 = 0u, h2 = 0u;
     for (uint32_t e = 4 * lane; e < stride; e += 256) {
       const float4 x = *reinterpret_cast<const float4 *>(row + e);
       const uint32_t c0 = screen_u8_code(x.x, lo, scale), c1 = screen_u8_code(x.y, lo, scale);
@@ -1115,7 +1254,28 @@
         sum = fmaf(d2, d2, sum);
         sum = fmaf(d3, d3, sum);
       }
-      *reinterpret_cast<uint32_t *>(dst + kScreenU8Header + e) = c0 | (c1 << 8) | (c2 << 16) | (c3 << 24);
+      const uint32_t w = c0 | (c1 << 8) | (c2 << 16) | (c3 << 24);
+      if constexpr (!kNib) {
+        *reinterpret_cast<uint32_t *>(dst + kScreenU8Header + e) = w;
+      } else {
+        const uint32_t wh = (w >> 4) & 0x0f0f0f0fu, wl = w & 0x0f0f0f0fu;
+        const uint32_t g0 = wh & 0xffu, g1 = (wh >> 8) & 0xffu, g2 = (wh >> 16) & 0xffu, g3 = wh >> 24;
+        h1 += (g0 + g1) + (g2 + g3);
+        h2 += (g0 * g0 + g1 * g1) + (g2 * g2 + g3 * g3);
+        const float f0 = x.x - screen_u8_value(g0, lo4, scale4), f1 = x.y - screen_u8_value(g1, lo4, scale4);
+        const float f2 = x.z - screen_u8_value(g2, lo4, scale4), f3 = x.w - screen_u8_value(g3, lo4, scale4);
+        if (!bad) {
+          sum4 = fmaf(f0, f0, sum4);
+          sum4 = fmaf(f1, f1, sum4);
+          sum4 = fmaf(f2, f2, sum4);
+          sum4 = fmaf(f3, f3, sum4);
+        }
+        const uint32_t ph = wh | (lane_xor<1>(wh) << 4), pl = wl | (lane_xor<1>(wl) << 4);
+        if ((lane & 1) == 0) {
+          *reinterpret_cast<uint32_t *>(dst + kScreenU8Header + e / 2) = ph;
+          *reinterpret_cast<uint32_t *>(out_low + (first + r) * rec + kScreenU8Header + e / 2) = pl;
+        }
+      }
     }
     sum += lane_xor<1>(sum);
     sum += lane_xor<2>(sum);
@@ -1130,7 +1290,24 @@
     s1 += lane_xor<16>(s1); s2 += lane_xor<16>(s2);
     s1 = read_lane(s1, 0) + read_lane(s1, 32);
     s2 = read_lane(s2, 0) + read_lane(s2, 32);
-    if (lane == 0) {
+    if constexpr (kNib) {
+      sum4 += lane_xor<1>(sum4); h1 += lane_xor<1>(h1); h2 += lane_xor<1>(h2);
+      sum4 += lane_xor<2>(sum4); h1 += lane_xor<2>(h1); h2 += lane_xor<2>(h2);
+      sum4 += lane_xor<4>(sum4); h1 += lane_xor<4>(h1); h2 += lane_xor<4>(h2);
+      sum4 += lane_xor<8>(sum4); h1 += lane_xor<8>(h1); h2 += lane_xor<8>(h2);
+      sum4 += lane_xor<16>(sum4); h1 += lane_xor<16>(h1); h2 += lane_xor<16>(h2);
+      sum4 = read_lane(sum4, 0) + read_lane(sum4, 32);
+      h1 = read_lane(h1, 0) + read_lane(h1, 32);
+      h2 = read_lane(h2, 0) + read_lane(h2, 32);
+      if (lane == 0) {
+        const bool bad4 = bad || !screen_finite(lo4) || !screen_finite(scale4);
+        uint8_t *dlo = out_low + (first + r) * rec;
+        *reinterpret_cast<float4 *>(dst) = make_float4(screen_u8_err(sum4, stride, bad4), lo4, scale4, 0.f);
+        *reinterpret_cast<uint2 *>(dst + screen_nib_sums_offset(stride)) = make_uint2(h1, h2);
+        *reinterpret_cast<float4 *>(dlo) = make_float4(screen_u8_err(sum, stride, bad), lo, scale, 0.f);
+        *reinterpret_cast<uint2 *>(dlo + screen_nib_sums_offset(stride)) = make_uint2(s1, s2);
+      }
+    } else if (lane == 0) {
       *reinterpret_cast<float4 *>(dst) = make_float4(screen_u8_err(sum, stride, bad), lo, scale, 0.f);
       *reinterpret_cast<uint2 *>(dst + screen_u8_sums_offset(stride)) = make_uint2(s1, s2);
     }
@@ -1416,7 +1593,17 @@
                                  uint8_t *out_recs, hipStream_t stream) {
   if (count == 0) return hipSuccess;
   const int grid = static_cast<int>(std::min<uint64_t>((count + 3) / 4, 16384));
-  hipLaunchKernelGGL(screen_rows_u8_kernel, dim3(grid), dim3(256), 0, stream, base, first, count, stride, out_recs);
+  hipLaunchKernelGGL(screen_rows_u8_kernel<false>, dim3(grid), dim3(256), 0, stream, base, first, count, stride, out_recs,
+                     static_cast<uint8_t *>(nullptr));
+  return hipGetLastError();
+}
+
+hipError_t launch_screen_rows_nib(const float *base, uint64_t first, uint64_t count, uint32_t stride,
+                                  uint8_t *out_high, uint8_t *out_low, hipStream_t stream) {
+  if (count == 0) return hipSuccess;
+  const int grid = static_cast<int>(std::min<uint64_t>((count + 3) / 4, 16384));
+  hipLaunchKernelGGL(screen_rows_u8_kernel<true>, dim3(grid), dim3(256), 0, stream, base, first, count, stride, out_high,
+                     out_low);
   return hipGetLastError();
 }
 
diff --git a/include/alaya_hip.h b/include/alaya_hip.h
--- a/include/alaya_hip.h
+++ b/include/alaya_hip.h
@@ -140,11 +140,17 @@
 int alaya_index_help_stats(alaya_index *ix, uint64_t *memo_dists, uint64_t *memo_expansions,
                            uint64_t *helper_rows);
 int alaya_index_screen_stats(alaya_index *ix, uint64_t *screened, uint64_t *screened_out);
+int alaya_index_nibble_stats(alaya_index *ix, uint64_t *stage1_out, uint64_t *stage2, uint64_t *low_searcher,
+                             uint64_t *low_scout);
 int alaya_screen_lower_bound(const float *d_tilde, const float *e_row, uint64_t n, uint32_t dim, float *out);
 int alaya_screen_u8_quantize(const float *rows, uint64_t n, uint32_t dim, uint8_t *codes, float *header,
                              float *values);
 int alaya_screen_int_bound(const float *queries, const float *rows, uint64_t n, uint32_t dim, float *d_in,
                            float *e_sum, float *bound, uint32_t *sums);
+int alaya_screen_nibble_record_bytes(uint32_t dim);
+int alaya_screen_nibble_quantize(const float *rows, uint64_t n, uint32_t dim, uint8_t *high, uint8_t *low);
+int alaya_screen_nibble_bound(const float *queries, const float *rows, uint64_t n, uint32_t dim, float *bound4,
+                              float *bound8, uint32_t *sums);
 int alaya_flat_ip_slack(int contraction, uint32_t k_acc, const float *q_norm2, const int *q_exp, uint64_t n,
                         float b_max, int base_exp, float *out);
 int alaya_flat_ip_proven(const float *kth_d, const float *cutoff, const float *slack, uint64_t n, uint8_t *out);
```
